# weisongwen/ToySLAM

Hardware: AMD Instinct MI355X
Metric: scan registrations/sec (100k-pt src vs 1M-pt target, 30 Newton iters) (higher is better)
Workload: dtype f32; 1 GPU; single 100k-pt source vs 1M-pt target, 1.0 m voxels, DIRECT7, 30 Newton passes (max_iterations 28, epsilon 1e-9), set U; target_points=1000000, search=DIRECT7, outer_passes=30

## Files before the change

include/ndt_mi355.h:

```cpp
#ifndef NDT_MI355_H_
#define NDT_MI355_H_

#include <stddef.h>
#include <stdint.h>

#ifdef __cplusplus
extern "C" {
#endif

typedef struct ndt_context* ndt_handle;

typedef enum {
  NDT_OK = 0,
  NDT_ERR_INVALID = 1,
  NDT_ERR_NO_DEVICE = 2,
  NDT_ERR_HIP = 3,
  NDT_ERR_GRID_OVERFLOW = 4,
  NDT_ERR_NO_INPUT = 5,
  NDT_ERR_COMM = 6
} ndt_status;

typedef enum { NDT_KDTREE = 0, NDT_DIRECT26 = 1, NDT_DIRECT7 = 2, NDT_DIRECT1 = 3 } ndt_search_method;

const char* ndt_last_error(void);
// ... 112 lines not shown
ndt_status ndt_pcd_read_xyz(const char* path, void* out, size_t capacity_points, size_t stride_bytes, size_t* n_points,
                            int* is_dense);
ndt_status ndt_pcd_write_xyz(const char* path, const void* pts, size_t n, size_t stride_bytes, int binary);

typedef struct ndt_pcd_sequence* ndt_pcd_sequence_handle;
ndt_status ndt_pcd_sequence_open(const char* directory, ndt_pcd_sequence_handle* out);
ndt_status ndt_pcd_sequence_poll(ndt_pcd_sequence_handle s, size_t loaded_clouds, size_t* n_new_files);
ndt_status ndt_pcd_sequence_next(ndt_pcd_sequence_handle s, const void** pts, size_t* n, int* is_dense, int* file_number);
ndt_status ndt_pcd_sequence_stage(ndt_pcd_sequence_handle s, int device);
ndt_status ndt_pcd_sequence_next_device(ndt_pcd_sequence_handle s, const void** d_pts, const void** host_pts, size_t* n, int* is_dense,
                                        int* file_number);
ndt_status ndt_pcd_sequence_next_cloud(ndt_pcd_sequence_handle s, ndt_cloud* cloud, const void** host_pts, size_t* n, int* is_dense,
                                       int* file_number);
void ndt_pcd_sequence_close(ndt_pcd_sequence_handle s);
int ndt_host_extract_file_number(const char* file_stem);
ndt_status ndt_host_repack_fields(const void* data, size_t n, size_t point_step, size_t off_x, size_t off_y, size_t off_z,
                                  void* out_xyz1, int* is_dense);

ndt_status ndt_align_batch(ndt_handle h, const void* pts, const size_t* offsets , size_t n_scans,
                           size_t stride_bytes, const float* guesses ,
                           float* final_transformations , int* has_converged,
                           int* final_num_iteration, double* transformation_probability);
ndt_status ndt_align_batch_device(ndt_handle h, const void* d_pts, const size_t* offsets, size_t n_scans,
                                  size_t stride_bytes, const float* guesses, float* final_transformations,
                                  int* has_converged, int* final_num_iteration, double* transformation_probability);

ndt_status ndt_set_batch_groups(ndt_handle h, int n_groups);

ndt_status ndt_align_pairs(ndt_handle h, const void* pts, const size_t* offsets , size_t n_clouds,
                           size_t stride_bytes, int is_dense, const int* pairs , size_t n_pairs,
                           const float* guesses , float* final_transformations ,
                           int* has_converged, int* final_num_iteration, double* transformation_probability);
ndt_status ndt_align_pairs_clouds(ndt_handle h, const ndt_cloud* clouds, size_t n_clouds, int is_dense, const int* pairs,
                                  size_t n_pairs, const float* guesses, float* final_transformations, int* has_converged,
                                  int* final_num_iteration, double* transformation_probability);
ndt_status ndt_pairs_grid_size(ndt_handle h, size_t cloud, size_t* n_leaves, size_t* n_valid);
ndt_status ndt_pairs_grid_info(ndt_handle h, size_t cloud, int* min_b , int* max_b , int* div_b );
ndt_status ndt_pairs_grid_dump(ndt_handle h, size_t cloud, int64_t* idx, int* nr_points, double* mean, double* cov,
                               double* icov, double* evals);
ndt_status ndt_pairs_fitness_scores(ndt_handle h, const float* transforms , double max_range,
                                    double* fitness );
ndt_status ndt_pairs_count(ndt_handle h, size_t* n_pairs);
ndt_status ndt_batch_fitness_scores(ndt_handle h, const void* pts, const size_t* offsets , size_t n_scans,
                                    size_t stride_bytes, const float* transforms , double max_range,
                                    double* fitness );
ndt_status ndt_batch_fitness_scores_device(ndt_handle h, const void* d_pts, const size_t* offsets, size_t n_scans,
                                           size_t stride_bytes, const float* transforms, double max_range, double* fitness);
ndt_status ndt_diag_fitness_launches(ndt_handle h, size_t* launches, size_t* max_blocks);

ndt_status ndt_grid_centroids(ndt_handle h, float* xyz1 , int64_t* idx , size_t capacity,
                              size_t* n);
ndt_status ndt_grid_centroids_cloud(ndt_handle h, ndt_cloud* out);
ndt_status ndt_get_centroid_fitness_score(ndt_handle h, double max_range, double* fitness);
ndt_status ndt_batch_centroid_fitness_scores(ndt_handle h, const void* pts, const size_t* offsets , size_t n_scans,
                                             size_t stride_bytes, const float* transforms , double max_range,
                                             double* fitness );
ndt_status ndt_batch_centroid_fitness_scores_device(ndt_handle h, const void* d_pts, const size_t* offsets, size_t n_scans,
                                                    size_t stride_bytes, const float* transforms, double max_range, double* fitness);
ndt_status ndt_diag_centroid_fitness(ndt_handle h, size_t* launches, size_t* excursion_passes, float* excursion, size_t* max_blocks);

ndt_status ndt_score_poses(ndt_handle h, const float* transforms , size_t n_poses, double* scores );
ndt_status ndt_diag_score_poses(ndt_handle h, size_t* launches, size_t* blocks);
ndt_status ndt_align_guesses(ndt_handle h, const float* guesses , size_t n_guesses, float* final_transformations,
                             int* has_converged, int* final_num_iteration, double* transformation_probability, int* best);
void ndt_host_pick_top(const double* scores, size_t n, size_t keep, int* idx_out , size_t* n_out);
ndt_status ndt_align_multistart(ndt_handle h, const float* candidates , size_t n_candidates, size_t keep,
                                int* picked, size_t* n_picked, float* final_transformations, int* has_converged,
                                int* final_num_iteration, double* transformation_probability, int* best);

#define NDT_COMM_ID_BYTES 128
ndt_status ndt_comm_get_unique_id(void* id_out );
ndt_status ndt_comm_init_rank(ndt_handle h, const void* id, int rank, int world_size);
ndt_status ndt_comm_destroy(ndt_handle h);
ndt_status ndt_comm_stats(ndt_handle h, int* rank, int* world_size, long long* n_collectives, int* lock_steps);
ndt_status ndt_align_batch_sharded(ndt_handle h, const void* pts, const size_t* offsets , size_t n_local,
                                   size_t first_scan, size_t total_scans, size_t stride_bytes,
                                   const float* guesses , float* final_transformations ,
                                   int* has_converged, int* final_num_iteration, double* transformation_probability);
ndt_status ndt_align_batch_sharded_device(ndt_handle h, const void* d_pts, const size_t* offsets, size_t n_local,
                                          size_t first_scan, size_t total_scans, size_t stride_bytes, const float* guesses,
                                          float* final_transformations, int* has_converged, int* final_num_iteration,
                                          double* transformation_probability);

#define NDT_EVAL_STRIDE 32
typedef int (*ndt_allreduce_fn)(void* buf, size_t n_doubles, int on_device, void* user);
ndt_status ndt_set_allreduce(ndt_handle h, ndt_allreduce_fn fn, void* user, int on_device);

ndt_status ndt_eval(ndt_handle h, const double* p, double* score, double* gradient, double* hessian,
                    double* mean_neighbors);
ndt_status ndt_eval_with_matrix(ndt_handle h, const float* T, const double* p, double* score, double* gradient,
                                double* hessian, double* mean_neighbors);
ndt_status ndt_eval_hessian_f64(ndt_handle h, const double* p, double* hessian);

ndt_status ndt_grid_size(ndt_handle h, size_t* n_leaves, size_t* n_valid);
ndt_status ndt_grid_info(ndt_handle h, int* min_b , int* max_b , int* div_b );
ndt_status ndt_grid_dump(ndt_handle h, int64_t* idx, int* nr_points, double* mean, double* cov, double* icov,
                         double* evals);

ndt_status ndt_profile_enable(ndt_handle h, int on);

ndt_status ndt_set_evaluation_path(ndt_handle h, int persistent);
ndt_status ndt_profile_read(ndt_handle h, int kind, long long* n_launches, double* total_ms, int reset);

ndt_status ndt_selftest_reduce(ndt_handle h, int n_blocks, double* block_sums);
ndt_status ndt_selftest_server_idle(ndt_handle h, const double* p, int stall_ms, int* served_after_stall, double* scores);

ndt_status ndt_diag_stamps(ndt_handle h, const double* p, unsigned long long* stamps, size_t* n_waves);

ndt_status ndt_diag_eval_plan(ndt_handle h, size_t n, int* ppb, int* fused_blocks, int* launch_blocks, int* server_blocks,
                              int* batch_blocks);

ndt_status ndt_host_grid_plan(long long n_cells, long long n_points, const int* div_b , int* bucket_form, int* n_buckets,
                              int* cells_per_bucket, int* pts_per_block, int* n_blocks, int* one_launch, int* wmax, int* lds_cap,
                              long long* lut_cells, int* compact_items, long long* compact_tiles, int* compact_prefix,
                              int* filter_buckets, int* filter_chunks);
ndt_status ndt_diag_grid_build(ndt_handle h, int* form, size_t* n_points, long long* n_cells, int* n_buckets, int* cells_per_bucket,
                               int* pts_per_block, int* n_blocks, int* wmax, int* lds_cap, long long* lut_cells, int* compact_items,
                               long long* compact_tiles, int* compact_prefix, int* compact_pending);

ndt_status ndt_diag_server_roundtrip(ndt_handle h, const double* p, int n_iter, double* us);
ndt_status ndt_diag_selfdrive(ndt_handle h, const double* p, int rounds, double* us);

void ndt_host_solve6(const double* H , const double* b , double* x );
void ndt_host_pose_to_matrix(const double* p , float* T );
void ndt_host_matrix_to_pose(const float* T , double* p );
void ndt_host_angle_derivatives(const double* p , float* j_ang , float* h_ang ,
                                double* j_ang_d , double* h_ang_d );
void ndt_host_gauss(float resolution, double outlier_ratio, double* d );
void ndt_host_thread_budget(int* affinity_cpus, double* quota_cpus, int* local_world_size);
void ndt_host_thread_plan(int affinity_cpus, double quota_cpus, int local_world_size, int* pool_threads, int* max_batch_groups);
typedef int (*ndt_eval_cb)(void* user, int kind, const float* T, const double* p, double* score, double* g, double* H);
ndt_status ndt_host_run_driver(ndt_eval_cb cb, void* user, size_t n_source, const float* guess, float resolution,
                               double step_size, double outlier_ratio, double trans_eps, int max_iter,
                               float* final_transformation, int* has_converged, int* final_num_iteration,
                               double* transformation_probability, int* n_evals, int* n_hessian_recomputes);

#ifdef __cplusplus
}
#endif
#endif
```

toyslam_amd/_lib.py:

```python
import ctypes as C
import os
import subprocess

_HERE = os.path.dirname(os.path.abspath(__file__))
LIB_PATH = os.path.join(_HERE, "libndt_mi355.so")
CSRC = os.path.join(_HERE, "csrc")

NDT_OK, NDT_ERR_INVALID, NDT_ERR_NO_DEVICE, NDT_ERR_HIP, NDT_ERR_GRID_OVERFLOW, NDT_ERR_NO_INPUT, NDT_ERR_COMM = range(7)
KDTREE, DIRECT26, DIRECT7, DIRECT1 = 0, 1, 2, 3
EVAL_STRIDE = 32
COMM_ID_BYTES = 128

ALLREDUCE_FN = C.CFUNCTYPE(C.c_int, C.c_void_p, C.c_size_t, C.c_int, C.c_void_p)
EVAL_CB = C.CFUNCTYPE(C.c_int, C.c_void_p, C.c_int, C.POINTER(C.c_float), C.POINTER(C.c_double),
                      C.POINTER(C.c_double), C.POINTER(C.c_double), C.POINTER(C.c_double))


class NdtError(RuntimeError):
    def __init__(self, status, msg):
        super().__init__("ndt_mi355 status %d: %s" % (status, msg))
        self.status = status


def build(force=False):
# ... 32 lines not shown
    "ndt_set_input_source_device": (C.c_int, [vp, vp, C.c_size_t, C.c_size_t]),
    "ndt_share_input_target": (C.c_int, [vp, vp]),
    "ndt_set_cu_partition": (C.c_int, [vp, C.c_int]),
    "ndt_get_cu_partition": (C.c_int, [vp, ip, ip]),
    "ndt_set_input_target_device_ref": (C.c_int, [vp, vp, C.c_size_t, C.c_int]),
    "ndt_set_input_source_device_ref": (C.c_int, [vp, vp, C.c_size_t]),
    "ndt_share_input_source": (C.c_int, [vp, vp]),
    "ndt_set_voxel_index": (C.c_int, [vp, C.c_int]),
    "ndt_align": (C.c_int, [vp, fp, fp, ip, ip, dp, vp, C.c_size_t]),
    "ndt_get_result": (C.c_int, [vp, fp, ip, ip, dp]),
    "ndt_get_output_device": (C.c_int, [vp, C.POINTER(vp), szp]),
    "ndt_get_stats": (C.c_int, [vp, ip, ip, dp]),
    "ndt_calculate_score": (C.c_int, [vp, vp, C.c_size_t, C.c_size_t, dp]),
    "ndt_voxel_grid_filter": (C.c_int, [vp, vp, C.c_size_t, C.c_size_t, C.c_int, C.c_float, vp, C.c_size_t, szp]),
    "ndt_voxel_grid_filter_device": (C.c_int, [vp, vp, C.c_size_t, C.c_size_t, C.c_int, C.c_float, vp, szp]),
    "ndt_get_fitness_score": (C.c_int, [vp, C.c_double, dp]),
    "ndt_map_clear": (C.c_int, [vp]),
    "ndt_map_update": (C.c_int, [vp, vp, C.c_size_t, C.c_size_t, C.c_int, fp, C.c_float, ip]),
    "ndt_map_update_device": (C.c_int, [vp, vp, C.c_size_t, C.c_size_t, C.c_int, fp, C.c_float, ip]),
    "ndt_map_size": (C.c_int, [vp, szp]),
    "ndt_map_get": (C.c_int, [vp, vp, C.c_size_t]),
    "ndt_map_get_device": (C.c_int, [vp, C.POINTER(C.c_void_p), szp]),
    "ndt_cloud_voxel_filter": (C.c_int, [vp, vp, C.c_size_t, C.c_size_t, C.c_int, C.c_float, C.c_int, C.POINTER(vp), ip]),
    "ndt_warm_up": (C.c_int, [vp, C.c_size_t]),
    "ndt_cloud_upload": (C.c_int, [vp, vp, C.c_size_t, C.c_size_t, C.POINTER(vp)]),
    "ndt_cloud_size": (C.c_int, [vp, szp]),
    "ndt_cloud_data": (C.c_int, [vp, C.POINTER(C.c_void_p), szp]),
    "ndt_cloud_download": (C.c_int, [vp, vp, vp, C.c_size_t]),
    "ndt_cloud_release": (None, [vp]),
    "ndt_set_input_source_cloud": (C.c_int, [vp, vp]),
    "ndt_set_input_target_cloud": (C.c_int, [vp, vp, C.c_int]),
    "ndt_map_update_cloud": (C.c_int, [vp, vp, C.c_int, fp, C.c_float, ip]),
    "ndt_map_update_clouds": (C.c_int, [vp, C.POINTER(vp), C.c_size_t, ip, fp, C.c_float, ip]),
    "ndt_map_update_batch": (C.c_int, [vp, vp, szp, C.c_size_t, C.c_size_t, ip, fp, C.c_float, C.c_int, ip]),
    "ndt_diag_map_batch": (C.c_int, [vp, szp, szp, szp]),
    "ndt_promote_source_to_target": (C.c_int, [vp, C.c_int]),
    "ndt_target_accumulate": (C.c_int, [vp, vp, C.c_size_t, C.c_size_t, C.c_int, fp]),
    "ndt_target_accumulate_device": (C.c_int, [vp, vp, C.c_size_t, C.c_size_t, C.c_int, fp]),
    "ndt_target_accumulate_cloud": (C.c_int, [vp, vp, C.c_int, fp]),
    "ndt_target_accumulate_clouds": (C.c_int, [vp, C.POINTER(vp), C.c_size_t, C.c_int, fp]),
    "ndt_target_accumulate_reset": (C.c_int, [vp]),
    "ndt_target_accumulated": (C.c_int, [vp, szp, szp, szp]),
    "ndt_diag_target_accumulate": (C.c_int, [vp, szp, szp, ip, ip, szp]),
    "ndt_target_accumulate_crop": (C.c_int, [vp, fp, fp]),
    "ndt_diag_target_crop": (C.c_int, [vp, szp, szp, szp, ip, szp]),
    "ndt_target_accumulate_export": (C.c_int, [vp, fp, fp, vp, C.c_size_t, szp]),
    "ndt_target_accumulate_import": (C.c_int, [vp, vp, C.c_size_t]),
    "ndt_target_accumulate_save": (C.c_int, [vp, fp, fp, C.c_char_p]),
    "ndt_target_accumulate_load": (C.c_int, [vp, C.c_char_p]),
    "ndt_diag_target_export": (C.c_int, [vp, szp, szp, szp]),
    "ndt_host_acc_blob_info": (C.c_int, [vp, C.c_size_t, fp, szp, ip, ip]),
    "ndt_host_acc_blob_checksum": (C.c_int, [vp, C.c_size_t, C.POINTER(C.c_uint64)]),
    "ndt_host_acc_pack_cell": (C.c_int, [C.c_int, C.c_int, C.c_int, C.POINTER(C.c_uint64)]),
    "ndt_host_acc_unpack_cell": (None, [C.c_uint64, ip, ip, ip]),
    "ndt_host_chain_pose": (None, [fp, fp, fp]),
    "ndt_host_lattice": (C.c_int, [C.c_float, fp, fp, ip, ip, ip, C.POINTER(C.c_longlong), C.c_int, C.c_longlong, ip]),
    "ndt_pcd_read_header": (C.c_int, [C.c_char_p, szp, ip, ip]),
    "ndt_pcd_read_xyz": (C.c_int, [C.c_char_p, vp, C.c_size_t, C.c_size_t, szp, ip]),
    "ndt_pcd_write_xyz": (C.c_int, [C.c_char_p, vp, C.c_size_t, C.c_size_t, C.c_int]),
    "ndt_align_batch": (C.c_int, [vp, vp, szp, C.c_size_t, C.c_size_t, fp, fp, ip, ip, dp]),
    "ndt_align_batch_device": (C.c_int, [vp, vp, szp, C.c_size_t, C.c_size_t, fp, fp, ip, ip, dp]),
    "ndt_set_allreduce": (C.c_int, [vp, ALLREDUCE_FN, vp, C.c_int]),
    "ndt_set_batch_groups": (C.c_int, [vp, C.c_int]),
    "ndt_align_pairs": (C.c_int, [vp, vp, szp, C.c_size_t, C.c_size_t, C.c_int, ip, C.c_size_t, fp, fp, ip, ip, dp]),
    "ndt_align_pairs_clouds": (C.c_int, [vp, C.POINTER(vp), C.c_size_t, C.c_int, ip, C.c_size_t, fp, fp, ip, ip, dp]),
    "ndt_pairs_grid_size": (C.c_int, [vp, C.c_size_t, szp, szp]),
    "ndt_pairs_grid_info": (C.c_int, [vp, C.c_size_t, ip, ip, ip]),
    "ndt_pairs_grid_dump": (C.c_int, [vp, C.c_size_t, C.POINTER(C.c_int64), ip, dp, dp, dp, dp]),
    "ndt_pairs_fitness_scores": (C.c_int, [vp, fp, C.c_double, dp]),
    "ndt_pairs_count": (C.c_int, [vp, szp]),
    "ndt_diag_fitness_launches": (C.c_int, [vp, szp, szp]),
    "ndt_batch_fitness_scores": (C.c_int, [vp, vp, szp, C.c_size_t, C.c_size_t, fp, C.c_double, dp]),
    "ndt_batch_fitness_scores_device": (C.c_int, [vp, vp, szp, C.c_size_t, C.c_size_t, fp, C.c_double, dp]),
    "ndt_grid_centroids": (C.c_int, [vp, fp, C.POINTER(C.c_int64), C.c_size_t, szp]),
    "ndt_grid_centroids_cloud": (C.c_int, [vp, C.POINTER(vp)]),
    "ndt_get_centroid_fitness_score": (C.c_int, [vp, C.c_double, dp]),
    "ndt_batch_centroid_fitness_scores": (C.c_int, [vp, vp, szp, C.c_size_t, C.c_size_t, fp, C.c_double, dp]),
    "ndt_batch_centroid_fitness_scores_device": (C.c_int, [vp, vp, szp, C.c_size_t, C.c_size_t, fp, C.c_double, dp]),
    "ndt_diag_centroid_fitness": (C.c_int, [vp, szp, szp, fp, szp]),
    "ndt_score_poses": (C.c_int, [vp, fp, C.c_size_t, dp]),
    "ndt_diag_score_poses": (C.c_int, [vp, szp, szp]),
    "ndt_align_guesses": (C.c_int, [vp, fp, C.c_size_t, fp, ip, ip, dp, ip]),
    "ndt_host_pick_top": (None, [dp, C.c_size_t, C.c_size_t, ip, szp]),
    "ndt_align_multistart": (C.c_int, [vp, fp, C.c_size_t, C.c_size_t, ip, szp, fp, ip, ip, dp, ip]),
    "ndt_align_batch_sharded": (C.c_int, [vp, vp, szp, C.c_size_t, C.c_size_t, C.c_size_t, C.c_size_t, fp, fp, ip, ip, dp]),
    "ndt_align_batch_sharded_device": (C.c_int, [vp, vp, szp, C.c_size_t, C.c_size_t, C.c_size_t, C.c_size_t, fp, fp, ip, ip, dp]),
    "ndt_comm_get_unique_id": (C.c_int, [vp]),
    "ndt_comm_init_rank": (C.c_int, [vp, vp, C.c_int, C.c_int]),
    "ndt_comm_destroy": (C.c_int, [vp]),
    "ndt_comm_stats": (C.c_int, [vp, ip, ip, C.POINTER(C.c_longlong), ip]),
    "ndt_eval": (C.c_int, [vp, dp, dp, dp, dp, dp]),
    "ndt_eval_with_matrix": (C.c_int, [vp, fp, dp, dp, dp, dp, dp]),
    "ndt_eval_hessian_f64": (C.c_int, [vp, dp, dp]),
    "ndt_grid_size": (C.c_int, [vp, szp, szp]),
    "ndt_grid_info": (C.c_int, [vp, ip, ip, ip]),
    "ndt_grid_dump": (C.c_int, [vp, C.POINTER(C.c_int64), ip, dp, dp, dp, dp]),
    "ndt_diag_stamps": (C.c_int, [vp, dp, C.POINTER(C.c_ulonglong), szp]),
    "ndt_diag_eval_plan": (C.c_int, [vp, C.c_size_t, ip, ip, ip, ip, ip]),
    "ndt_host_grid_plan": (C.c_int, [C.c_longlong, C.c_longlong, ip, ip, ip, ip, ip, ip, ip, ip, ip, C.POINTER(C.c_longlong), ip,
                                     C.POINTER(C.c_longlong), ip, ip, ip]),
    "ndt_diag_grid_build": (C.c_int, [vp, ip, szp, C.POINTER(C.c_longlong), ip, ip, ip, ip, ip, ip, C.POINTER(C.c_longlong), ip,
                                      C.POINTER(C.c_longlong), ip, ip]),
    "ndt_diag_server_roundtrip": (C.c_int, [vp, dp, C.c_int, dp]),
    "ndt_diag_selfdrive": (C.c_int, [vp, dp, C.c_int, dp]),
    "ndt_selftest_reduce": (C.c_int, [vp, C.c_int, dp]),
    "ndt_selftest_server_idle": (C.c_int, [vp, dp, C.c_int, ip, dp]),
    "ndt_profile_enable": (C.c_int, [vp, C.c_int]),
    "ndt_set_evaluation_path": (C.c_int, [vp, C.c_int]),
    "ndt_profile_read": (C.c_int, [vp, C.c_int, C.POINTER(C.c_longlong), dp, C.c_int]),
    "ndt_host_solve6": (None, [dp, dp, dp]),
    "ndt_host_pose_to_matrix": (None, [dp, fp]),
    "ndt_host_matrix_to_pose": (None, [fp, dp]),
    "ndt_host_angle_derivatives": (None, [dp, fp, fp, dp, dp]),
    "ndt_host_gauss": (None, [C.c_float, C.c_double, dp]),
    "ndt_host_thread_budget": (None, [ip, dp, ip]),
    "ndt_host_thread_plan": (None, [C.c_int, C.c_double, C.c_int, ip, ip]),
    "ndt_host_run_driver": (C.c_int, [EVAL_CB, vp, C.c_size_t, fp, C.c_float, C.c_double, C.c_double, C.c_double,
                                      C.c_int, fp, ip, ip, dp, ip, ip]),
    "ndt_pcd_sequence_open": (C.c_int, [C.c_char_p, C.POINTER(vp)]),
    "ndt_pcd_sequence_poll": (C.c_int, [vp, C.c_size_t, szp]),
    "ndt_pcd_sequence_next": (C.c_int, [vp, C.POINTER(vp), szp, ip, ip]),
    "ndt_pcd_sequence_close": (None, [vp]),
    "ndt_pcd_sequence_stage": (C.c_int, [vp, C.c_int]),
    "ndt_pcd_sequence_next_cloud": (C.c_int, [vp, C.POINTER(vp), C.POINTER(C.c_void_p), szp, ip, ip]),
    "ndt_cloud_voxel_filter_begin": (C.c_int, [vp, vp, C.c_int, C.c_float]),
    "ndt_cloud_voxel_filter_end": (C.c_int, [vp, C.POINTER(vp), ip]),
    "ndt_cloud_voxel_filter_batch": (C.c_int, [vp, vp, szp, C.c_size_t, C.c_size_t, ip, C.c_float, C.c_int, C.POINTER(vp), ip]),
    "ndt_cloud_voxel_filter_clouds": (C.c_int, [vp, C.POINTER(vp), C.c_size_t, ip, C.c_float, C.POINTER(vp), ip]),
    "ndt_diag_filter_batch": (C.c_int, [vp, szp, szp, szp]),
    "ndt_pcd_sequence_next_device": (C.c_int, [vp, C.POINTER(C.c_void_p), C.POINTER(C.c_void_p), szp, ip, ip]),
    "ndt_host_extract_file_number": (C.c_int, [C.c_char_p]),
    "ndt_host_repack_fields": (C.c_int, [vp, C.c_size_t, C.c_size_t, C.c_size_t, C.c_size_t, C.c_size_t, vp, ip]),
    "gicp_create": (C.c_int, [C.c_int, C.POINTER(vp)]),
    "gicp_destroy": (None, [vp]),
    "gicp_set_correspondence_randomness": (C.c_int, [vp, C.c_int]),
    "gicp_set_rotation_epsilon": (C.c_int, [vp, C.c_double]),
    "gicp_set_maximum_optimizer_iterations": (C.c_int, [vp, C.c_int]),
    "gicp_set_transformation_epsilon": (C.c_int, [vp, C.c_double]),
    "gicp_set_maximum_iterations": (C.c_int, [vp, C.c_int]),
    "gicp_set_max_correspondence_distance": (C.c_int, [vp, C.c_double]),
    "gicp_set_input_target": (C.c_int, [vp, vp, C.c_size_t, C.c_size_t]),
    "gicp_set_input_source": (C.c_int, [vp, vp, C.c_size_t, C.c_size_t]),
    "gicp_set_source_covariances": (C.c_int, [vp, dp, C.c_size_t]),
    "gicp_set_target_covariances": (C.c_int, [vp, dp, C.c_size_t]),
    "gicp_set_input_target_cloud": (C.c_int, [vp, vp]),
    "gicp_set_input_source_cloud": (C.c_int, [vp, vp]),
    "gicp_align_pairs_clouds": (C.c_int, [vp, C.POINTER(vp), C.c_size_t, ip, C.c_size_t, fp, C.c_double, fp, ip, ip, ip, dp]),
    "gicp_align_pairs_lockstep": (C.c_int, [vp, C.POINTER(vp), C.c_size_t, ip, C.c_size_t, fp, C.c_double, fp, ip, ip, ip, dp]),
    "gicp_align_guesses": (C.c_int, [vp, fp, C.c_size_t, C.c_double, fp, ip, ip, ip, dp]),
    "gicp_diag_lockstep": (C.c_int, [vp, szp, szp, szp, szp]),
    "gicp_pairs_covariances": (C.c_int, [vp, C.c_size_t, dp]),
    "gicp_diag_pairs": (C.c_int, [vp, szp, szp, szp]),
    "gicp_diag_pairs_time": (C.c_int, [vp, dp, dp]),
    "gicp_align": (C.c_int, [vp, fp, fp, ip, ip, vp]),
    "gicp_get_result": (C.c_int, [vp, fp, ip, ip]),
    "gicp_get_fitness_score": (C.c_int, [vp, C.c_double, dp]),
    "gicp_get_stats": (C.c_int, [vp, ip, ip, ip, ip]),
    "gicp_covariances": (C.c_int, [vp, C.c_int, dp, ip, fp]),
    "gicp_step_correspond": (C.c_int, [vp, fp, fp, ip, fp, ip]),
    "gicp_step_functor": (C.c_int, [vp, C.c_int, dp, dp, dp]),
    "gicp_diag_plan": (C.c_int, [vp, C.c_size_t, ip]),
    "gicp_host_apply_state": (None, [dp, fp]),
}


def lib():
# ... 19 lines not shown
```

toyslam_amd/csrc/ndt_batch.hip:

```cpp
#include "ndt_internal.hpp"

#include <condition_variable>
#include <dlfcn.h>
#include <sched.h>
#include <rccl/rccl.h>

namespace ndtc {

class StepPool {
 public:
  explicit StepPool(int n_threads) : n_(std::max(1, n_threads)) {
    for (int t = 1; t < n_; t++) workers_.emplace_back([this, t] { loop(t); });
  }
  ~StepPool() {
    stop_.store(true, std::memory_order_release);
    post();
    for (auto& w : workers_) w.join();
  }
  template <class F>
  void run(size_t count, const F& fn) {
    if (n_ == 1 || count < 32) {
      for (size_t i = 0; i < count; i++) fn(i);
      return;
    }
// ... 131 lines not shown
  Rccl* r = rccl();
  return fail(NDT_ERR_COMM, std::string(what) + " failed: " + (r ? r->GetErrorString(e) : "librccl unavailable"));
}

void comm_release(ndt_context* h) {
  if (!h->comm) return;
  if (Rccl* r = rccl()) (void)r->CommDestroy(static_cast<ncclComm_t>(h->comm));
  h->comm = nullptr;
  h->comm_rank = 0;
  h->comm_world = 1;
}

ndt_status comm_allreduce(ndt_context* h, double* d_buf, size_t n) {
  Rccl* r = rccl();
  if (!r || !h->comm) return fail(NDT_ERR_COMM, "no communicator");
  const ncclResult_t e = r->AllReduce(d_buf, d_buf, n, ncclDouble, ncclSum, static_cast<ncclComm_t>(h->comm), h->stream);
  if (e != ncclSuccess) return rccl_fail("ncclAllReduce", e);
  h->comm_collectives++;
  return NDT_OK;
}

static int poll_timeout_s() {
  static const int v = [] { const char* e = getenv("NDT_BATCH_TIMEOUT_S"); return e ? std::max(1, atoi(e)) : 60; }();
  return v;
}

template <class LiveFn>
static ndt_status poll_rows(ndt_context* h, size_t n_rows, unsigned long long seq, const LiveFn& live) {
  const auto t0 = std::chrono::steady_clock::now();
  unsigned spins = 0;
  for (size_t k = 0; k < n_rows; k++) {
    if (!live(k)) continue;
    volatile unsigned long long* flag = reinterpret_cast<volatile unsigned long long*>(h->host_result + k * ndt::kEvalStride) + (ndt::kEvalStride - 1);
    while (__atomic_load_n(flag, __ATOMIC_ACQUIRE) != seq) {
      __builtin_ia32_pause();
      if ((++spins & 0xFFFF) == 0) {
        if (hipStreamQuery(h->stream) != hipErrorNotReady) {
          HIP_TRY(hipStreamSynchronize(h->stream));
          if (__atomic_load_n(flag, __ATOMIC_ACQUIRE) == seq) break;
          return fail(NDT_ERR_HIP, "batch step finished without publishing its results");
        }
        if (std::chrono::steady_clock::now() - t0 > std::chrono::seconds(poll_timeout_s())) {
          if (h->comm) {
            Rccl* r = rccl();
            if (r && r->CommAbort) (void)r->CommAbort(static_cast<ncclComm_t>(h->comm));
            h->comm = nullptr;
            h->comm_rank = 0;
            h->comm_world = 1;
            return fail(NDT_ERR_COMM, "timed out waiting for the exchange step (a rank never joined the all-reduce); communicator aborted");
          }
          return fail(NDT_ERR_HIP, "timed out waiting for the batch step");
        }
      }
    }
  }
  return NDT_OK;
}

}

extern "C" {

static ndt_status align_batch_impl(ndt_handle h, const void* pts, const size_t* offsets, size_t n_local, size_t stride,
                                   bool on_device, const float* guesses, float* final_T, int* conv, int* iters,
                                   double* tprob, size_t first = 0, size_t total = 0) {
  if (!h || !offsets) return fail(NDT_ERR_INVALID, "bad arguments");
  if (!h->grid || !h->target) return fail(NDT_ERR_NO_INPUT, "no input target");
  const bool sharded = total != 0;
  if (!sharded) total = n_local;
  if (first + n_local > total) return fail(NDT_ERR_INVALID, "scan range outside the batch");
  const bool exchange = h->comm != nullptr || h->allreduce != nullptr;
  if (sharded && n_local != total && !exchange)
    return fail(NDT_ERR_COMM, "a sharded batch needs a communicator (ndt_comm_init_rank) or an all-reduce hook");
  if (total == 0) return NDT_OK;
  if (total > 65535) return fail(NDT_ERR_INVALID, "at most 65535 scans per batch");
  for (size_t k = 0; k < n_local; k++)
    if (offsets[k + 1] < offsets[k]) return fail(NDT_ERR_INVALID, "offsets must be non-decreasing");
  ndt_status s = ensure_device(h);
  if (s) return s;
  if (!h->is_batch_worker) {
    s = maybe_compact_records(h, true);
    if (s) return s;
  }
  std::shared_ptr<DeviceCloud> cloud;
  const size_t n_pts = n_local ? offsets[n_local] - offsets[0] : 0;
  const unsigned char* base = n_local ? static_cast<const unsigned char*>(pts) + offsets[0] * stride : nullptr;
  s = upload_cloud(h, base, n_pts, stride, on_device, cloud);
  if (s) return s;
  if (n_local) {
    s = order_cloud(h, cloud.get(), offsets, n_local);
    if (s) return s;
  }
  const bool use_sorted = cloud->n_sorted > 0 && !cloud->scan_counts.empty();
  LockStepMembers m;
  m.pts = use_sorted ? cloud->sorted.p : cloud->pts.p;
  m.offset.resize(n_local);
  m.count.resize(n_local);
  m.n_raw.resize(n_local);
  for (size_t k = 0; k < n_local; k++) {
    m.n_raw[k] = offsets[k + 1] - offsets[k];
    m.offset[k] = static_cast<int>(use_sorted ? cloud->scan_starts[k] : offsets[k] - offsets[0]);
    m.count[k] = static_cast<int>(use_sorted ? cloud->scan_counts[k] : m.n_raw[k]);
  }
  return lock_step(h, m, n_local, guesses, final_T, conv, iters, tprob, first, sharded ? total : 0);
}

}

namespace ndtc {

ndt_status lock_step(ndt_context* h, const LockStepMembers& m, size_t n_local, const float* guesses, float* final_T, int* conv,
                     int* iters, double* tprob, size_t first, size_t total) {
  const bool sharded = total != 0;
  if (!sharded) total = n_local;
  const bool exchange = h->comm != nullptr || h->allreduce != nullptr;
  if (m.views && (sharded || exchange)) return fail(NDT_ERR_INVALID, "per-member grids are not sharded");
  const float4* batch_pts = m.pts;
  ndt_status s = ensure_host_rows(h, total);
  if (s) return s;
  HIP_TRY(h->batch_out.reserve(total * ndt::kEvalStride));
  const ndt::Gauss gs = ndt::gauss_constants(h->resolution, h->outlier_ratio);
  auto is_local = [&](size_t g) { return g >= first && g < first + n_local; };

  auto exchange_rows = [&](const std::function<bool(size_t)>& live) -> ndt_status {
    if (h->comm) {
      ndt_status sc = comm_allreduce(h, h->batch_out.p, total * ndt::kEvalStride);
      if (sc) return sc;
      if (h->profiling) HIP_TRY(hipEventRecord(h->ev_c, h->stream));
      const unsigned long long seq = ++h->eval_seq;
      HIP_TRY(ndt::launch_publish_rows(h->batch_out.p, static_cast<int>(total), h->host_result, seq, h->stream));
      if (h->profiling) HIP_TRY(hipEventRecord(h->ev_d, h->stream));
      return poll_rows(h, total, seq, live);
    }
    if (h->allreduce_on_device) {
      HIP_TRY(hipStreamSynchronize(h->stream));
      if (h->allreduce(h->batch_out.p, total * ndt::kEvalStride, 1, h->allreduce_user)) return fail(NDT_ERR_COMM, "allreduce callback failed");
    }
    HIP_TRY(hipMemcpyAsync(h->host_result, h->batch_out.p, total * ndt::kEvalStride * sizeof(double), hipMemcpyDeviceToHost, h->stream));
    HIP_TRY(hipStreamSynchronize(h->stream));
    if (!h->allreduce_on_device && h->allreduce(h->host_result, total * ndt::kEvalStride, 0, h->allreduce_user))
      return fail(NDT_ERR_COMM, "allreduce callback failed");
    return NDT_OK;
  };

  std::vector<size_t> counts(total, 0);
  for (size_t k = 0; k < n_local; k++) counts[first + k] = m.n_raw[k];
  if (sharded && exchange) {
    std::vector<double> rows(total * ndt::kEvalStride, 0.0);
    for (size_t k = 0; k < n_local; k++) rows[(first + k) * ndt::kEvalStride] = static_cast<double>(counts[first + k]);
    HIP_TRY(hipMemcpyAsync(h->batch_out.p, rows.data(), rows.size() * sizeof(double), hipMemcpyHostToDevice, h->stream));
    HIP_TRY(hipStreamSynchronize(h->stream));
    s = exchange_rows([](size_t) { return true; });
    if (s) return s;
    for (size_t g = 0; g < total; g++) counts[g] = static_cast<size_t>(h->host_result[g * ndt::kEvalStride]);
  }

  std::vector<ndt::ScanSolver> solvers(total);
  const size_t pinned_need = (total * sizeof(ndt::ScanDesc) + 4 * total * sizeof(int) + 15) & ~static_cast<size_t>(15);
  if (pinned_need > h->batch_pinned_bytes) {
    if (h->batch_pinned) (void)hipHostFree(h->batch_pinned);
    h->batch_pinned = nullptr;
    h->batch_pinned_bytes = 0;
    HIP_TRY(hipHostMalloc(&h->batch_pinned, pinned_need, hipHostMallocDefault));
    h->batch_pinned_bytes = pinned_need;
  }
  ndt::ScanDesc* descs = static_cast<ndt::ScanDesc*>(h->batch_pinned);
  int* active = reinterpret_cast<int*>(descs + total);
  std::vector<int> live_kind(total, ndt::EVAL_NONE);
  size_t max_n = 0;
  for (size_t g = 0; g < total; g++) {
    solvers[g].start(guesses ? guesses + 16 * g : nullptr, counts[g], solver_params(h));
    descs[g].offset = 0;
    descs[g].count = 0;
    descs[g].pad = 0;
// ... 175 lines not shown
    if (tprob) tprob[g] = solvers[g].trans_probability;
  }
  return NDT_OK;
}

}

extern "C" {

static ndt_status align_batch_grouped(ndt_handle h, const void* pts, const size_t* offsets, size_t n_scans, size_t stride,
                                      bool on_device, const float* guesses, float* final_T, int* conv, int* iters,
                                      double* tprob) {
  const bool exchange = h && (h->comm != nullptr || h->allreduce != nullptr);
  const size_t groups = batch_group_count(h, n_scans);
  if (!h || !offsets || exchange || groups <= 1 || !h->grid || !h->target || h->profiling)
    return align_batch_impl(h, pts, offsets, n_scans, stride, on_device, guesses, final_T, conv, iters, tprob);
  ndt_status s0 = ensure_device(h);
  if (s0) return s0;
  s0 = maybe_compact_records(h, true);
  if (s0) return s0;
  return run_groups(
      h, n_scans, groups, [&](size_t lo, size_t hi) { return static_cast<double>(offsets[hi] - offsets[lo]); },
      [&](ndt_context* w, size_t lo, size_t hi) {
        return align_batch_impl(w, pts, offsets + lo, hi - lo, stride, on_device, guesses ? guesses + 16 * lo : nullptr,
                                final_T ? final_T + 16 * lo : nullptr, conv ? conv + lo : nullptr, iters ? iters + lo : nullptr,
                                tprob ? tprob + lo : nullptr);
      });
}

}

namespace ndtc {

ndt_status many_poses_checks(const ndt_context* h, const void* table, size_t n, const void* out, const char* what) {
  if (!h) return fail(NDT_ERR_INVALID, "null handle");
  if (n && (!table || !out)) return fail(NDT_ERR_INVALID, std::string("null ") + what);
  if (h->comm || h->allreduce)
    return fail(NDT_ERR_INVALID, "one source under many poses is not sharded: the handle has a communicator or an all-reduce hook");
  return NDT_OK;
}

size_t batch_group_count(const ndt_context* h, size_t n_scans) {
  static const int forced = [] { const char* v = getenv("NDT_BATCH_GROUPS"); return v ? std::max(1, atoi(v)) : 0; }();
  size_t groups = (h && h->batch_groups_wanted > 0) ? static_cast<size_t>(h->batch_groups_wanted)
                  : forced                           ? static_cast<size_t>(forced)
                                                     : (n_scans >= 192 ? 4 : n_scans >= 16 ? 2 : 1);
  groups = std::min(groups, std::max<size_t>(1, n_scans / 4));
  static const int max_groups = [] {
    int aff = 1, lw = 1, mg = 1;
    double quota = 0;
    host_thread_budget(&aff, &quota, &lw);
    host_thread_plan(aff, quota, lw, nullptr, &mg);
    return mg;
  }();
  if (!(h && h->batch_groups_wanted > 0) && !forced) groups = std::min(groups, static_cast<size_t>(max_groups));
  return groups;
}

ndt_status run_groups(ndt_context* h, size_t n_scans, size_t groups, const std::function<double(size_t, size_t)>& pts_of,
                      const std::function<ndt_status(ndt_context*, size_t, size_t)>& run) {
  HIP_TRY(hipStreamSynchronize(h->stream));
  while (h->batch_workers.size() < groups) {
    ndt_context* w = new ndt_context();
    w->device = h->device;
    w->is_batch_worker = true;
    h->batch_workers.push_back(w);
  }
  std::vector<ndt_status> st(groups, NDT_OK);
  std::vector<std::string> msg(groups);
  std::vector<std::thread> threads;
  for (size_t g = 0; g < groups; g++) {
    ndt_context* w = h->batch_workers[g];
    w->resolution = h->resolution;
    w->step_size = h->step_size;
    w->outlier_ratio = h->outlier_ratio;
    w->trans_eps = h->trans_eps;
    w->max_iter = h->max_iter;
    w->search = h->search;
    w->min_pts = h->min_pts;
    w->eig_ratio = h->eig_ratio;
    w->target = h->target;
    w->target_dense = h->target_dense;
    w->grid = h->grid;
    const size_t lo = n_scans * g / groups, hi = n_scans * (g + 1) / groups;
    threads.emplace_back([=, &st, &msg, &run] {
      ndt_status s = run(w, lo, hi);
      st[g] = s;
      if (s) msg[g] = ndt_last_error();
    });
  }
  for (auto& t : threads) t.join();
  for (size_t g = 0; g < groups; g++) {
    ndt_context* w = h->batch_workers[g];
    if (w->stream) (void)hipStreamSynchronize(w->stream);
    w->target.reset();
    w->grid.reset();
  }
  long long ne = 0, nh = 0;
  double nn_w = 0, pts_w = 0;
  int steps = 0;
  for (size_t g = 0; g < groups; g++) {
    ndt_context* w = h->batch_workers[g];
    if (st[g]) return fail(st[g], msg[g]);
    const size_t lo = n_scans * g / groups, hi = n_scans * (g + 1) / groups;
    const double evals_pts = static_cast<double>(w->n_evals) * (hi > lo ? pts_of(lo, hi) / static_cast<double>(hi - lo) : 0.0);
    ne += w->n_evals;
    nh += w->n_hess;
    nn_w += w->mean_neighbors * evals_pts;
    pts_w += evals_pts;
    steps = std::max(steps, w->batch_lock_steps);
  }
  h->n_evals = static_cast<int>(std::min<long long>(ne, INT32_MAX));
  h->n_hess = static_cast<int>(std::min<long long>(nh, INT32_MAX));
  h->mean_neighbors = pts_w > 0 ? nn_w / pts_w : 0.0;
  h->batch_lock_steps = steps;
  h->batch_groups = static_cast<int>(groups);
  return NDT_OK;
}

}

extern "C" {

ndt_status ndt_align_batch(ndt_handle h, const void* pts, const size_t* offsets, size_t n_scans, size_t stride,
                           const float* guesses, float* final_T, int* conv, int* iters, double* tprob) {
  return align_batch_grouped(h, pts, offsets, n_scans, stride, false, guesses, final_T, conv, iters, tprob);
}
ndt_status ndt_align_batch_device(ndt_handle h, const void* pts, const size_t* offsets, size_t n_scans, size_t stride,
                                  const float* guesses, float* final_T, int* conv, int* iters, double* tprob) {
  return align_batch_grouped(h, pts, offsets, n_scans, stride, true, guesses, final_T, conv, iters, tprob);
}
ndt_status ndt_align_batch_sharded(ndt_handle h, const void* pts, const size_t* offsets, size_t n_local, size_t first_scan,
                                   size_t total_scans, size_t stride, const float* guesses, float* final_T, int* conv, int* iters,
                                   double* tprob) {
  if (total_scans == 0) return fail(NDT_ERR_INVALID, "total_scans must be > 0");
  return align_batch_impl(h, pts, offsets, n_local, stride, false, guesses, final_T, conv, iters, tprob, first_scan, total_scans);
}
ndt_status ndt_align_batch_sharded_device(ndt_handle h, const void* d_pts, const size_t* offsets, size_t n_local, size_t first_scan,
                                          size_t total_scans, size_t stride, const float* guesses, float* final_T, int* conv,
                                          int* iters, double* tprob) {
  if (total_scans == 0) return fail(NDT_ERR_INVALID, "total_scans must be > 0");
  return align_batch_impl(h, d_pts, offsets, n_local, stride, true, guesses, final_T, conv, iters, tprob, first_scan, total_scans);
}

ndt_status ndt_align_guesses(ndt_handle h, const float* guesses, size_t n_guesses, float* final_T, int* conv, int* iters,
                             double* tprob, int* best) {
  ndt_status s = many_poses_checks(h, guesses, n_guesses, h, "guesses");
  if (s) return s;
  if (n_guesses > 65535) return fail(NDT_ERR_INVALID, "at most 65535 guesses per call");
  if (n_guesses == 0) {
    if (best) *best = -1;
    return NDT_OK;
  }
  s = ensure_device(h);
  if (s) return s;
  if (!h->grid || !h->target) return fail(NDT_ERR_NO_INPUT, "no input target");
  if (!h->source) return fail(NDT_ERR_NO_INPUT, "no input source");
  s = maybe_compact_records(h, true);
  if (s) return s;
  const DeviceCloud& src = *h->source;
  DeviceCloud view;
  LockStepMembers m;
  m.pts = src.pts.p;
  int count = static_cast<int>(src.n);
  if (src.n_sorted > 0) {
    m.pts = src.sorted.p;
    count = static_cast<int>(src.n_sorted);
  } else if (src.n > 0) {
    view.pts.borrow(src.pts.p, src.n);
    view.n = src.n;
    const size_t offsets[2] = {0, src.n};
    s = order_cloud(h, &view, offsets, 1);
    if (s) return s;
    if (view.n_sorted > 0 && !view.scan_counts.empty()) {
      m.pts = view.sorted.p + view.scan_starts[0];
      count = static_cast<int>(view.scan_counts[0]);
    }
  }
  m.offset.assign(n_guesses, 0);
  m.count.assign(n_guesses, count);
  m.n_raw.assign(n_guesses, src.n);
  std::vector<double> tp(n_guesses, 0.0);
  s = lock_step(h, m, n_guesses, guesses, final_T, conv, iters, tp.data());
  if (s) return s;
  if (tprob) std::memcpy(tprob, tp.data(), n_guesses * sizeof(double));
  if (best) {
    *best = -1;
    for (size_t g = 0; g < n_guesses; g++)
      if (!std::isnan(tp[g]) && (*best < 0 || tp[g] > tp[*best])) *best = static_cast<int>(g);
  }
  return NDT_OK;
}

void ndt_host_pick_top(const double* scores, size_t n, size_t keep, int* idx_out, size_t* n_out) {
  std::vector<int> idx;
  for (size_t i = 0; scores && i < n; i++)
    if (std::isfinite(scores[i])) idx.push_back(static_cast<int>(i));
  const size_t k = std::min(keep, idx.size());
  std::partial_sort(idx.begin(), idx.begin() + k, idx.end(),
                    [&](int a, int b) { return scores[a] > scores[b] || (scores[a] == scores[b] && a < b); });
  for (size_t i = 0; idx_out && i < k; i++) idx_out[i] = idx[i];
  if (n_out) *n_out = k;
}

ndt_status ndt_align_multistart(ndt_handle h, const float* candidates, size_t n_candidates, size_t keep, int* picked,
                                size_t* n_picked, float* final_T, int* conv, int* iters, double* tprob, int* best) {
  ndt_status s = many_poses_checks(h, candidates, n_candidates, h, "candidates");
  if (s) return s;
  if (n_candidates > static_cast<size_t>(std::numeric_limits<int>::max())) return fail(NDT_ERR_INVALID, "too many candidates");
  if (std::min(keep, n_candidates) > 65535) return fail(NDT_ERR_INVALID, "at most 65535 guesses are registered per call");
  if (n_picked) *n_picked = 0;
  if (best) *best = -1;
  if (n_candidates == 0 || keep == 0) return NDT_OK;
  std::vector<double> scores(n_candidates);
  s = ndt_score_poses(h, candidates, n_candidates, scores.data());
  if (s) return s;
  std::vector<int> idx(std::min(keep, n_candidates));
  size_t np = 0;
  ndt_host_pick_top(scores.data(), n_candidates, keep, idx.data(), &np);
  if (np == 0) return NDT_OK;
  std::vector<float> guesses(16 * np);
  for (size_t k = 0; k < np; k++) std::memcpy(guesses.data() + 16 * k, candidates + 16 * static_cast<size_t>(idx[k]), 16 * sizeof(float));
  int b = -1;
  s = ndt_align_guesses(h, guesses.data(), np, final_T, conv, iters, tprob, &b);
  if (s) return s;
// ... 79 lines not shown
```

toyslam_amd/csrc/ndt_clouds.hip:

```cpp
#include "ndt_internal.hpp"

#include <immintrin.h>

namespace ndtc {

static void host_repack_bbox(const unsigned char* src, size_t n, size_t stride, float* dst, float bb_min[2][3], float bb_max[2][3]) {
  __m128 mn0 = _mm_set1_ps(FLT_MAX), mx0 = _mm_set1_ps(-FLT_MAX), mn1 = mn0, mx1 = mx0;
  const __m128 keep_xyz = _mm_castsi128_ps(_mm_set_epi32(0, -1, -1, -1)), one_w = _mm_set_ps(1.0f, 0.0f, 0.0f, 0.0f);
  const __m128 abs_mask = _mm_castsi128_ps(_mm_set1_epi32(0x7fffffff)), inf = _mm_set1_ps(INFINITY);
  auto take = [&](__m128 v, float* out) {
    v = _mm_or_ps(_mm_and_ps(v, keep_xyz), one_w);
    _mm_store_ps(out, v);
    mn0 = _mm_min_ps(v, mn0);
    mx0 = _mm_max_ps(v, mx0);
    if ((_mm_movemask_ps(_mm_cmplt_ps(_mm_and_ps(v, abs_mask), inf)) & 7) == 7) {
      mn1 = _mm_min_ps(v, mn1);
      mx1 = _mm_max_ps(v, mx1);
    }
  };
  const size_t n_wide = (stride >= 16) ? n : (n ? n - 1 : 0);
  for (size_t i = 0; i < n_wide; i++) take(_mm_loadu_ps(reinterpret_cast<const float*>(src + i * stride)), dst + 4 * i);
  for (size_t i = n_wide; i < n; i++) {
    const float* p = reinterpret_cast<const float*>(src + i * stride);
    take(_mm_set_ps(0.0f, p[2], p[1], p[0]), dst + 4 * i);
// ... 173 lines not shown

BBox bbox_of(const DeviceCloud& c, int dense) {
  BBox b;
  const int v = dense ? 0 : 1;
  for (int k = 0; k < 3; k++) {
    b.mn[k] = c.bb_min[v][k];
    b.mx[k] = c.bb_max[v][k];
  }
  return b;
}
ndt_status bbox_compute(ndt_context* h, const float4* d_pts, int n, int dense, BBox& out) {
  const int nb = std::min(1024, (n + 255) / 256);
  DevBuf<float> d_mm;
  HIP_TRY(d_mm.reserve(static_cast<size_t>(nb) * 6));
  HIP_TRY(ndt::launch_bbox(d_pts, n, dense, d_mm.p, nb, h->stream));
  std::vector<float> mm(static_cast<size_t>(nb) * 6);
  HIP_TRY(hipMemcpyAsync(mm.data(), d_mm.p, mm.size() * sizeof(float), hipMemcpyDeviceToHost, h->stream));
  HIP_TRY(hipStreamSynchronize(h->stream));
  for (int k = 0; k < 3; k++) {
    out.mn[k] = FLT_MAX;
    out.mx[k] = -FLT_MAX;
  }
  for (int b = 0; b < nb; b++)
    for (int k = 0; k < 3; k++) {
      out.mn[k] = std::min(out.mn[k], mm[b * 6 + k]);
      out.mx[k] = std::max(out.mx[k], mm[b * 6 + 3 + k]);
    }
  return NDT_OK;
}

ndt_status order_range(ndt_context* h, const float4* d_pts, size_t n, float pitch, float4* d_out, size_t* n_out,
                       const BBox* known_bbox) {
  *n_out = 0;
  if (n == 0) return NDT_OK;
  hipStream_t st = h->stream;
  const int ni = static_cast<int>(n);
  BBox bb;
  if (known_bbox) bb = *known_bbox;
  else { ndt_status sb = bbox_compute(h, d_pts, ni, 0, bb); if (sb) return sb; }
  const float* min_p = bb.mn;
  const float* max_p = bb.mx;
  if (!(min_p[0] <= max_p[0])) return NDT_OK;
  ndt::GridGeom geo{};
  while (ndt::lattice_geometry(pitch, min_p, max_p, geo) != ndt::kLatticeOk || geo.n_cells > 4000000) pitch *= 2.0f;
  static const bool radix_on = [] { const char* v = getenv("NDT_ORDER"); return !v || std::strcmp(v, "chain") != 0; }();
  static const size_t radix_from = [] { const char* v = getenv("NDT_ORDER_RADIX_FROM"); return v ? static_cast<size_t>(std::max(0, atoi(v))) : static_cast<size_t>(65536); }();
  if (radix_on && n >= radix_from && ndt::order_radix_passes(geo.n_cells) <= 3) {
    int digit_bits = 0;
    const size_t words = ndt::order_radix_cntmat_words(geo.n_cells, ni, nullptr, nullptr, &digit_bits);
    const int passes = ndt::order_radix_passes(geo.n_cells);
    DevBuf<unsigned> cntmat, bucket_base, counts;
    DevBuf<float4> tmp;
    HIP_TRY(cntmat.reserve(words));
    HIP_TRY(bucket_base.reserve((static_cast<size_t>(1) << digit_bits) + 1));
    HIP_TRY(counts.reserve(4));
    if (passes > 1) HIP_TRY(tmp.reserve(n));
    HIP_TRY(ndt::launch_order_radix(d_pts, ni, geo, cntmat.p, bucket_base.p, tmp.p, d_out, counts.p, st));
    unsigned kept = 0;
    HIP_TRY(hipMemcpyAsync(&kept, counts.p + (passes - 1), sizeof(kept), hipMemcpyDeviceToHost, st));
    HIP_TRY(hipStreamSynchronize(st));
    *n_out = kept;
    return NDT_OK;
  }
  DevBuf<unsigned> cell_count, totals, rank;
  DevBuf<int> key;
  ChainBufs lv;
  HIP_TRY(cell_count.reserve(static_cast<size_t>(geo.n_cells)));
  HIP_TRY(key.reserve(n));
  HIP_TRY(rank.reserve(n));
  HIP_TRY(hipMemsetAsync(cell_count.p, 0, static_cast<size_t>(geo.n_cells) * sizeof(unsigned), st));
  HIP_TRY(ndt::launch_count(d_pts, ni, 0, geo, key.p, rank.p, cell_count.p, st));
  const size_t n_leaves = std::min<size_t>(n, static_cast<size_t>(geo.n_cells));
  HIP_TRY(totals.reserve(4));
  HIP_TRY(lv.reserve(n_leaves, n));
  if (ndt_status s = chain_scan_scatter(st, cell_count.p, geo.n_cells, 1, key.p, rank.p, ni, lv.out(), totals.p)) return s;
  HIP_TRY(ndt::launch_sort_gather(d_pts, lv.leaf_start.p, lv.leaf_count.p, static_cast<int>(n_leaves), lv.sorted_idx.p, d_out, st, totals.p));
  unsigned tot[3];
  HIP_TRY(hipMemcpyAsync(tot, totals.p, sizeof(tot), hipMemcpyDeviceToHost, st));
  HIP_TRY(hipStreamSynchronize(st));
  *n_out = tot[0];
  return NDT_OK;
}

ndt_status order_batch(ndt_context* h, DeviceCloud* c, const size_t* offsets, size_t n_scans) {
  hipStream_t st = h->stream;
  c->scan_counts.assign(n_scans, 0);
  c->scan_starts.assign(n_scans + 1, 0);
  c->n_sorted = 0;
  if (n_scans == 0 || c->n == 0) return NDT_OK;
  constexpr double kMaxCounters = 32.0e6;
  std::vector<int> off(n_scans + 1);
  size_t max_scan = 0;
  for (size_t k = 0; k <= n_scans; k++) off[k] = static_cast<int>(offsets[k] - offsets[0]);
  for (size_t k = 0; k < n_scans; k++) max_scan = std::max(max_scan, offsets[k + 1] - offsets[k]);
  DevBuf<int> d_off, d_box;
  HIP_TRY(d_off.reserve(n_scans + 1));
  HIP_TRY(d_box.reserve(6 * n_scans));
  std::vector<int> box(6 * n_scans);
  for (size_t k = 0; k < n_scans; k++)
    for (int j = 0; j < 6; j++) box[6 * k + j] = j < 3 ? std::numeric_limits<int>::max() : std::numeric_limits<int>::min();
  HIP_TRY(hipMemcpyAsync(d_off.p, off.data(), (n_scans + 1) * sizeof(int), hipMemcpyHostToDevice, st));
  HIP_TRY(hipMemcpyAsync(d_box.p, box.data(), box.size() * sizeof(int), hipMemcpyHostToDevice, st));
  HIP_TRY(ndt::launch_scan_bboxes(c->pts.p, d_off.p, static_cast<int>(n_scans), static_cast<int>(max_scan), d_box.p, st));
  HIP_TRY(hipMemcpyAsync(box.data(), d_box.p, box.size() * sizeof(int), hipMemcpyDeviceToHost, st));
  HIP_TRY(hipStreamSynchronize(st));
  std::vector<ndt::ScanLattice> lat(n_scans);
  for (size_t k = 0; k < n_scans; k++) {
    ndt::ScanLattice& L = lat[k];
    L = ndt::ScanLattice{};
    if (box[6 * k] > box[6 * k + 3]) continue;
    float mn[3], mx[3];
    for (int j = 0; j < 3; j++) { mn[j] = ndt::scan_bbox_decode(box[6 * k + j]); mx[j] = ndt::scan_bbox_decode(box[6 * k + 3 + j]); }
    for (float pitch = h->resolution;; pitch *= 2.0f) {
      const float inv = 1.0f / pitch;
      double cells = 1;
      int div[3];
      for (int j = 0; j < 3; j++) {
        L.min_b[j] = static_cast<int>(std::floor(mn[j] * inv));
        div[j] = static_cast<int>(std::floor(mx[j] * inv)) - L.min_b[j] + 1;
        cells *= div[j];
      }
      if (cells <= kMaxCounters) {
        L.inv_leaf = inv;
        L.mul1 = div[0];
        L.mul2 = div[0] * div[1];
        L.n_cells = static_cast<int>(cells);
        break;
      }
    }
  }
  DevBuf<unsigned> cell_count, totals, rank, d_starts;
  DevBuf<int> key;
  ChainBufs lv;
  DevBuf<ndt::ScanLattice> d_lat;
  DevBuf<long long> d_bases;
  size_t out_base = 0;
  for (size_t s0 = 0; s0 < n_scans;) {
    size_t ns = 0;
    long long total_cells = 0;
    while (s0 + ns < n_scans && (ns == 0 || static_cast<double>(total_cells + lat[s0 + ns].n_cells) <= kMaxCounters)) {
      lat[s0 + ns].base = total_cells;
      total_cells += lat[s0 + ns].n_cells;
      ns++;
    }
    const size_t first_pt = offsets[s0] - offsets[0], n_pts = offsets[s0 + ns] - offsets[s0];
    if (n_pts == 0 || total_cells == 0) {
      for (size_t k = 0; k < ns; k++) c->scan_starts[s0 + k] = out_base;
      s0 += ns;
      continue;
    }
    const int ni = static_cast<int>(n_pts);
    const float4* in = c->pts.p + first_pt;
    std::vector<int> poff(ns + 1);
    std::vector<long long> bases(ns + 1);
    size_t pass_max = 0;
    for (size_t k = 0; k <= ns; k++) poff[k] = static_cast<int>(offsets[s0 + k] - offsets[s0]);
    for (size_t k = 0; k < ns; k++) {
      pass_max = std::max(pass_max, offsets[s0 + k + 1] - offsets[s0 + k]);
      bases[k] = lat[s0 + k].base;
    }
    bases[ns] = total_cells;
    HIP_TRY(d_off.reserve(ns + 1));
    HIP_TRY(d_lat.reserve(ns));
    HIP_TRY(d_bases.reserve(ns + 1));
    HIP_TRY(d_starts.reserve(ns + 1));
    HIP_TRY(hipMemcpyAsync(d_off.p, poff.data(), (ns + 1) * sizeof(int), hipMemcpyHostToDevice, st));
    HIP_TRY(hipMemcpyAsync(d_lat.p, lat.data() + s0, ns * sizeof(ndt::ScanLattice), hipMemcpyHostToDevice, st));
    HIP_TRY(hipMemcpyAsync(d_bases.p, bases.data(), (ns + 1) * sizeof(long long), hipMemcpyHostToDevice, st));
    HIP_TRY(cell_count.reserve(static_cast<size_t>(total_cells) + 1));
    HIP_TRY(key.reserve(n_pts));
    HIP_TRY(rank.reserve(n_pts));
    HIP_TRY(hipMemsetAsync(cell_count.p, 0, (static_cast<size_t>(total_cells) + 1) * sizeof(unsigned), st));
    HIP_TRY(ndt::launch_count_batch(in, d_off.p, static_cast<int>(ns), static_cast<int>(pass_max), d_lat.p, key.p, rank.p, cell_count.p, st));
    const long long scan_cells = total_cells + 1;
    const size_t n_leaves = std::min<size_t>(n_pts, static_cast<size_t>(scan_cells));
    HIP_TRY(totals.reserve(4));
    HIP_TRY(lv.reserve(n_leaves, n_pts));
    if (ndt_status s = chain_scan(st, cell_count.p, scan_cells, 1, lv.out(), totals.p)) return s;
    unsigned tot[3];
    HIP_TRY(hipMemcpyAsync(tot, totals.p, sizeof(tot), hipMemcpyDeviceToHost, st));
    std::vector<unsigned> starts(ns + 1);
    HIP_TRY(ndt::launch_pick(cell_count.p, d_bases.p, d_starts.p, static_cast<int>(ns + 1), st));
    HIP_TRY(hipMemcpyAsync(starts.data(), d_starts.p, (ns + 1) * sizeof(unsigned), hipMemcpyDeviceToHost, st));
    HIP_TRY(ndt::launch_scatter(key.p, rank.p, ni, cell_count.p, lv.sorted_idx.p, st));
    HIP_TRY(ndt::launch_sort_gather(in, lv.leaf_start.p, lv.leaf_count.p, static_cast<int>(n_leaves), lv.sorted_idx.p, c->sorted.p + out_base, st, totals.p));
    HIP_TRY(hipStreamSynchronize(st));
    for (size_t k = 0; k < ns; k++) {
      c->scan_starts[s0 + k] = out_base + starts[k];
      c->scan_counts[s0 + k] = starts[k + 1] - starts[k];
    }
    out_base += starts[ns];
    c->n_sorted += tot[0];
    s0 += ns;
  }
  c->scan_starts[n_scans] = out_base;
  return NDT_OK;
}

ndt_status order_cloud(ndt_context* h, DeviceCloud* c, const size_t* offsets, size_t n_scans) {
  static const int mode = [] { const char* v = getenv("NDT_SORT_SOURCE"); return v ? (atoi(v) != 0 ? 1 : 0) : -1; }();
  constexpr size_t kOrderFrom = 65536;
  c->n_sorted = 0;
  const bool enabled = mode < 0 ? (offsets != nullptr || c->n >= kOrderFrom) : mode != 0;
  if (!enabled || c->n == 0) return NDT_OK;
  HIP_TRY(c->sorted.reserve(c->n));
  if (!offsets) {
    size_t got = 0;
    const BBox bb = bbox_of(*c, 0);
    ndt_status s = order_range(h, c->pts.p, c->n, h->resolution, c->sorted.p, &got, &bb);
    if (s) return s;
    c->n_sorted = got;
  } else {
    ndt_status s = order_batch(h, c, offsets, n_scans);
    if (s) return s;
  }
  return NDT_OK;
}

ndt_status cloud_use_on(ndt_handle h, DeviceCloud* c) {
  if (c->made_on && c->made_on != h->stream) {
    if (c->device != h->device) return fail(NDT_ERR_INVALID, "the cloud lives on another device");
    if (!DevPool::instance().retired(c->made_on)) HIP_TRY(hipStreamSynchronize(c->made_on));
    if (std::find(c->used_on.begin(), c->used_on.end(), h->stream) == c->used_on.end()) c->used_on.push_back(h->stream);
  }
  return NDT_OK;
}

}

extern "C" {

static ndt_status set_source_impl(ndt_handle h, const void* pts, size_t n, size_t stride, bool on_device, bool by_ref = false) {
  if (!h) return fail(NDT_ERR_INVALID, "null handle");
  std::shared_ptr<DeviceCloud> c;
  ndt_status s = upload_cloud(h, pts, n, stride, on_device, c, by_ref);
  if (s) return s;
  s = order_cloud(h, c.get(), nullptr, 0);
  if (s) return s;
  h->source = c;
  return NDT_OK;
}
ndt_status ndt_set_input_source(ndt_handle h, const void* pts, size_t n, size_t stride) {
  return set_source_impl(h, pts, n, stride, false);
}
ndt_status ndt_set_input_source_device(ndt_handle h, const void* pts, size_t n, size_t stride) {
  return set_source_impl(h, pts, n, stride, true);
}
ndt_status ndt_set_input_source_device_ref(ndt_handle h, const void* d_pts, size_t n) {
  return set_source_impl(h, d_pts, n, sizeof(float4), true, true);
}

ndt_status ndt_share_input_source(ndt_handle dst, ndt_handle src) {
  if (!dst || !src) return fail(NDT_ERR_INVALID, "null handle");
  if (!src->source) return fail(NDT_ERR_NO_INPUT, "the donor handle has no input source");
  if (dst == src) return NDT_OK;
  if (dst->device != src->device) return fail(NDT_ERR_INVALID, "handles on different devices");
  HIP_TRY(hipSetDevice(src->device));
  if (src->device_ready) HIP_TRY(hipStreamSynchronize(src->stream));
  ndt_status s = ensure_device(dst);
  if (s) return s;
  HIP_TRY(hipStreamSynchronize(dst->stream));
  dst->source = src->source;
  return NDT_OK;
}

ndt_status ndt_cloud_upload(ndt_handle h, const void* pts, size_t n, size_t stride, ndt_cloud* out) {
  if (!h || !out) return fail(NDT_ERR_INVALID, "bad arguments");
  *out = nullptr;
  std::shared_ptr<DeviceCloud> c;
  ndt_status s = upload_cloud(h, pts, n, stride, false, c);
  if (s) return s;
  c->device = h->device;
  c->made_on = h->stream;
  *out = new ndt_cloud_s{c};
  return NDT_OK;
}

ndt_status ndt_cloud_size(ndt_cloud c, size_t* n) {
  if (!c || !n) return fail(NDT_ERR_INVALID, "bad arguments");
  *n = c->c->n;
  return NDT_OK;
}
ndt_status ndt_cloud_data(ndt_cloud c, const void** d_pts, size_t* n) {
  if (!c || !d_pts || !n) return fail(NDT_ERR_INVALID, "bad arguments");
  *d_pts = c->c->pts.p;
  *n = c->c->n;
  return NDT_OK;
}
ndt_status ndt_cloud_download(ndt_handle h, ndt_cloud c, void* out, size_t out_stride) {
  if (!h || !c || (c->c->n && !out)) return fail(NDT_ERR_INVALID, "bad arguments");
  if (out_stride < 16) return fail(NDT_ERR_INVALID, "out_stride_bytes must be >= 16");
  ndt_status s = ensure_device(h);
  if (!s) s = cloud_use_on(h, c->c.get());
  if (s) return s;
  return download_records(h, c->c->pts.p, c->c->n, out, out_stride);
}
void ndt_cloud_release(ndt_cloud c) { delete c; }

ndt_status ndt_set_input_source_cloud(ndt_handle h, ndt_cloud c) {
// ... 22 lines not shown
```

toyslam_amd/csrc/ndt_grid_kernels.hip:

```cpp
#include "ndt_device.hpp"
#include "ndt_voxel_finish.hpp"

namespace ndt {

namespace {

__global__ __launch_bounds__(kBlock) void k_repack(const unsigned char* __restrict__ src, size_t n, size_t stride,
                                                   float4* __restrict__ dst) {
  for (size_t i = blockIdx.x * (size_t)kBlock + threadIdx.x; i < n; i += (size_t)gridDim.x * kBlock) {
    const float* p = reinterpret_cast<const float*>(src + i * stride);
    dst[i] = make_float4(p[0], p[1], p[2], 1.0f);
  }
}

__global__ __launch_bounds__(kBlock) void k_bbox(const float4* __restrict__ pts, int n, int dense,
                                                 float* __restrict__ block_minmax) {
  float mn[3] = {FLT_MAX, FLT_MAX, FLT_MAX}, mx[3] = {-FLT_MAX, -FLT_MAX, -FLT_MAX};
  for (int i = blockIdx.x * kBlock + threadIdx.x; i < n; i += gridDim.x * kBlock) {
    const float4 p = pts[i];
    if (!dense && !finite3(p.x, p.y, p.z)) continue;
    mn[0] = fminf(mn[0], p.x); mx[0] = fmaxf(mx[0], p.x);
    mn[1] = fminf(mn[1], p.y); mx[1] = fmaxf(mx[1], p.y);
    mn[2] = fminf(mn[2], p.z); mx[2] = fmaxf(mx[2], p.z);
  }
// ... 681 lines not shown
  if (lane == kWave - 1) lds[wave] = inc;
  __syncthreads();
  unsigned base = 0, total = 0;
  for (int w = 0; w < nthreads / kWave; w++) {
    if (w < wave) base += lds[w];
    total += lds[w];
  }
  unsigned run = base + inc - sum;
  for (int i = lo; i < hi; i++) {
    const unsigned v = agent_loads ? __hip_atomic_load(src + i, __ATOMIC_RELAXED, __HIP_MEMORY_SCOPE_AGENT) : src[i];
    dst[i] = run;
    run += v;
  }
  if (tid == 0) dst[n] = total;
}

constexpr int kMatchSlots = 256;
__device__ __forceinline__ unsigned wave_rank(int key, bool valid, unsigned long long* mtab, unsigned short* row, int bits) {
  const int lane = threadIdx.x & (kWave - 1);
  unsigned long long* slot = mtab + (key & (kMatchSlots - 1));
  if (valid) (void)__hip_atomic_fetch_or(slot, 1ull << lane, __ATOMIC_RELAXED, __HIP_MEMORY_SCOPE_WORKGROUP);
  const unsigned long long slotmask = valid ? __hip_atomic_load(slot, __ATOMIC_RELAXED, __HIP_MEMORY_SCOPE_WORKGROUP) : 0ull;
  const unsigned old = valid ? row[key] : 0u;
  unsigned long long peers = slotmask;
#pragma unroll
  for (int b = 8; b < 14; b++) {
    if (b < bits) {
      const bool bit = ((key >> b) & 1) != 0;
      const unsigned long long m = __ballot(bit);
      peers &= bit ? m : ~m;
    }
  }
  const unsigned first_of_slot = __builtin_amdgcn_mbcnt_hi(static_cast<unsigned>(slotmask >> 32), __builtin_amdgcn_mbcnt_lo(static_cast<unsigned>(slotmask), 0u));
  if (valid && first_of_slot == 0) __hip_atomic_store(slot, 0ull, __ATOMIC_RELAXED, __HIP_MEMORY_SCOPE_WORKGROUP);
  const unsigned below = __builtin_amdgcn_mbcnt_hi(static_cast<unsigned>(peers >> 32), __builtin_amdgcn_mbcnt_lo(static_cast<unsigned>(peers), 0u));
  if (valid && below == 0) row[key] = static_cast<unsigned short>(old + static_cast<unsigned>(__popcll(peers)));
  return old + below;
}

__global__ __launch_bounds__(kK1Threads) void k1_hist(const float4* __restrict__ pts, int n, int dense, GridGeom g, int map, int K,
                                                      int ppb, unsigned* __restrict__ cntmat, int* __restrict__ lut, long long lut_cells,
                                                      const unsigned* __restrict__ n_dev) {
  extern __shared__ unsigned k1_lds[];
  if (n_dev) n = min(n, static_cast<int>(*n_dev));
  const K1Deal deal(map & 255, map >> 8);
  unsigned* h = k1_lds;
  const int slice = k1_slice(blockIdx.x, gridDim.x);
  const int lo = min(static_cast<long long>(n), static_cast<long long>(slice) * ppb), hi = min(static_cast<long long>(n), static_cast<long long>(lo) + ppb);
  float4 p[8];
#pragma unroll
  for (int u = 0; u < 8; u++) {
    const int i = lo + threadIdx.x + u * kK1Threads;
    p[u] = (i < hi) ? pts[i] : make_float4(NAN, NAN, NAN, 0.f);
  }
  for (int k = threadIdx.x; k < K; k += kK1Threads) h[k] = 0;
  {
    const long long n4 = lut_cells / 4, per = (n4 + gridDim.x - 1) / gridDim.x;
    const long long lo4 = static_cast<long long>(blockIdx.x) * per, hi4 = min(n4, lo4 + per);
    int4* l4 = reinterpret_cast<int4*>(lut);
    for (long long i = lo4 + threadIdx.x; i < hi4; i += kK1Threads) l4[i] = make_int4(kLutEmpty, kLutEmpty, kLutEmpty, kLutEmpty);
    if (blockIdx.x == 0)
      for (long long i = n4 * 4 + threadIdx.x; i < lut_cells; i += kK1Threads) lut[i] = kLutEmpty;
  }
  __syncthreads();
  for (int base = lo + threadIdx.x; base < hi; base += 8 * kK1Threads) {
    if (base != lo + static_cast<int>(threadIdx.x)) {
#pragma unroll
      for (int u = 0; u < 8; u++) {
        const int i = base + u * kK1Threads;
        p[u] = (i < hi) ? pts[i] : make_float4(NAN, NAN, NAN, 0.f);
      }
    }
#pragma unroll
    for (int u = 0; u < 8; u++) {
      const int c = (base + u * kK1Threads < hi) ? key_of(g, p[u], dense) : -1;
      if (c >= 0) atomicAdd(&h[k1_bucket(c, deal)], 1u);
    }
  }
  __syncthreads();
  for (int k = threadIdx.x; k < K; k += kK1Threads) cntmat[static_cast<size_t>(slice) * K + k] = h[k];
}

constexpr int kColCols = 16, kColGroups = kK1Threads / kColCols, kColRows = 32;
__global__ __launch_bounds__(kK1Threads) void k1_colscan(unsigned* __restrict__ cntmat, int B, int K, unsigned* __restrict__ total) {
  __shared__ unsigned s_part[kColGroups][kColCols + 1];
  const int c = threadIdx.x % kColCols, rg = threadIdx.x / kColCols;
  const int col = blockIdx.x * kColCols + c;
  const int R = (B + kColGroups - 1) / kColGroups;
  const int r0 = rg * R;
  unsigned v[kColRows];
  unsigned sum = 0;
#pragma unroll
  for (int i = 0; i < kColRows; i++) {
    const int r = r0 + i;
    v[i] = (i < R && r < B && col < K) ? cntmat[static_cast<size_t>(r) * K + col] : 0u;
  }
#pragma unroll
  for (int i = 0; i < kColRows; i++) sum += v[i];
  s_part[rg][c] = sum;
  __syncthreads();
  unsigned base = 0, all = 0;
  for (int gq = 0; gq < kColGroups; gq++) {
    const unsigned t = s_part[gq][c];
    if (gq < rg) base += t;
    all += t;
  }
#pragma unroll
  for (int i = 0; i < kColRows; i++) {
    const int r = r0 + i;
    if (i < R && r < B && col < K) cntmat[static_cast<size_t>(r) * K + col] = base;
    base += v[i];
  }
  if (rg == 0 && col < K) total[col] = all;
}

__global__ __launch_bounds__(kK1Threads) void k1_scatter(const float4* __restrict__ pts, int n, int dense, GridGeom g, int map, int K,
                                                         int ppb, const unsigned* __restrict__ cntmat, const unsigned* __restrict__ total,
                                                         unsigned* __restrict__ bucket_base, float4* __restrict__ bpts,
                                                         unsigned* __restrict__ counts, unsigned long long* __restrict__ st, int index_form,
                                                         const unsigned* __restrict__ n_dev) {
  extern __shared__ unsigned k1_lds[];
  if (n_dev) n = min(n, static_cast<int>(*n_dev));
  const K1Deal deal(map & 255, map >> 8);
  __shared__ unsigned s_scan[kK1Waves];
  auto mark = [&](int q) {
    if (st && threadIdx.x == 0) st[8 * blockIdx.x + q] = stamp();
  };
  mark(0);
  __shared__ unsigned long long s_mtab[kK1Waves * kMatchSlots];
  unsigned long long* mtab_all = s_mtab;
  unsigned* cursor = k1_lds;
  unsigned short* tot = reinterpret_cast<unsigned short*>(cursor + K + 2);
  unsigned short* tab = tot + K;
  const int lane = threadIdx.x & (kWave - 1), wave = threadIdx.x / kWave;
  const int b = k1_slice(blockIdx.x, gridDim.x);
  const int kbits = k1_key_bits(K);
  const int lo = min(static_cast<long long>(n), static_cast<long long>(b) * ppb), hi = min(static_cast<long long>(n), static_cast<long long>(lo) + ppb);
  float4 p[8];
#pragma unroll
  for (int u = 0; u < 8; u++) {
    const int i = lo + wave * (8 * kWave) + u * kWave + lane;
    p[u] = (i < hi) ? pts[i] : make_float4(NAN, NAN, NAN, 0.f);
  }
  for (int i = threadIdx.x; i < kK1Waves * kMatchSlots; i += kK1Threads) mtab_all[i] = 0ull;
  for (int i = threadIdx.x; i < kK1Waves * K / 2; i += kK1Threads) reinterpret_cast<unsigned*>(tab)[i] = 0u;
  block_scan_array(total, cursor, K, kK1Threads, s_scan, false);
  __syncthreads();
  if (b == 0) {
    for (int k = threadIdx.x; k <= K; k += kK1Threads) bucket_base[k] = cursor[k];
    if (threadIdx.x == 0) counts[0] = cursor[K];
  }
  for (int k = threadIdx.x; k < K; k += kK1Threads) cursor[k] += cntmat[static_cast<size_t>(b) * K + k];
  __syncthreads();
  mark(1);
  unsigned short* row = tab + wave * K;
  unsigned long long* mtab = mtab_all + wave * kMatchSlots;
  for (int r0 = lo; r0 < hi; r0 += kK1Round) {
    int key[8];
    unsigned rk[8];
    if (r0 != lo) {
#pragma unroll
      for (int u = 0; u < 8; u++) {
        const int i = r0 + wave * (8 * kWave) + u * kWave + lane;
        p[u] = (i < hi) ? pts[i] : make_float4(NAN, NAN, NAN, 0.f);
      }
    }
#pragma unroll
    for (int u = 0; u < 8; u++) {
      const int i = r0 + wave * (8 * kWave) + u * kWave + lane;
      const int c = (i < hi) ? key_of(g, p[u], dense) : -1;
      key[u] = (c >= 0) ? k1_bucket(c, deal) : -1;
      rk[u] = 0;
      if (r0 + wave * (8 * kWave) + u * kWave < hi) rk[u] = wave_rank(key[u], key[u] >= 0, mtab, row, kbits);
    }
    __syncthreads();
    if (r0 == lo) mark(2);
    for (int k = threadIdx.x; k < K; k += kK1Threads) {
      unsigned s_ = 0;
#pragma unroll
      for (int w = 0; w < kK1Waves; w++) {
        const unsigned t = tab[w * K + k];
        tab[w * K + k] = static_cast<unsigned short>(s_);
        s_ += t;
      }
      tot[k] = static_cast<unsigned short>(s_);
    }
    __syncthreads();
    if (r0 == lo) mark(3);
#pragma unroll
    for (int u = 0; u < 8; u++) {
      if (key[u] >= 0) {
        const int i = r0 + wave * (8 * kWave) + u * kWave + lane;
        const unsigned pos = cursor[key[u]] + row[key[u]] + rk[u];
        if (index_form) reinterpret_cast<int*>(bpts)[pos] = i;
        else bpts[pos] = make_float4(p[u].x, p[u].y, p[u].z, __int_as_float(i));
      }
    }
    __syncthreads();
    if (r0 == lo) mark(4);
    if (r0 + kK1Round < hi) {
      for (int k = threadIdx.x; k < K; k += kK1Threads) cursor[k] += tot[k];
      for (int i = threadIdx.x; i < kK1Waves * K / 2; i += kK1Threads) reinterpret_cast<unsigned*>(tab)[i] = 0u;
      __syncthreads();
    }
  }
}

struct K1GlobalSrc {
  const float4* __restrict__ p;
  const int* __restrict__ idx;
  __device__ __forceinline__ float4 operator()(unsigned j) const {
    if (idx) {
      const int i = idx[j];
      float4 q = p[i];
      q.w = __int_as_float(i);
      return q;
    }
    return p[j];
  }
};
__device__ __forceinline__ K1GlobalSrc k1_src(const float4* bpts, const float4* cloud, unsigned bb) {
  return cloud ? K1GlobalSrc{cloud, reinterpret_cast<const int*>(bpts) + bb} : K1GlobalSrc{bpts + bb, nullptr};
}
template <class Src>
__device__ __forceinline__ void k1_cell_histogram(const Src& src, unsigned nb, const GridGeom& g,
                                                  const K1Deal& deal, int C, unsigned* cnt) {
  for (int c = threadIdx.x; c < C; c += kBlock) cnt[c] = 0;
  __syncthreads();
  for (unsigned j = threadIdx.x; j < nb; j += kBlock) {
    const float4 p = src(j);
    atomicAdd(&cnt[k1_local(build_cell(g, p.x, p.y, p.z), deal)], 1u);
  }
  __syncthreads();
}

__global__ __launch_bounds__(kBlock) void k1_count(const float4* __restrict__ bpts, GridGeom g, int map, int K, int C, unsigned min_pts,
                                                   const unsigned* __restrict__ bucket_base, unsigned* __restrict__ tot,
                                                   unsigned* __restrict__ ticket, unsigned* __restrict__ occ_base,
                                                   unsigned* __restrict__ cand_base, unsigned* __restrict__ counts, const float4* __restrict__ cloud) {
  extern __shared__ unsigned k1_lds[];
  const K1Deal deal(map & 255, map >> 8);
  __shared__ U3 s_u3[kBlock / kWave];
  __shared__ unsigned s_scan[kBlock / kWave];
  __shared__ int s_last;
  const int k = blockIdx.x;
  const unsigned bb = bucket_base[k], be = bucket_base[k + 1];
  U3 t = {0, 0, 0};
  if (be > bb) {
    k1_cell_histogram(k1_src(bpts, cloud, bb), be - bb, g, deal, C, k1_lds);
    for (int c = threadIdx.x; c < C; c += kBlock) {
      const unsigned v = k1_lds[c];
      t.occ += (v > 0);
      t.cand += (v >= min_pts);
    }
  }
  U3 total;
  block_exclusive_scan(t, total, s_u3);
  if (threadIdx.x == 0) {
    __hip_atomic_store(tot + 2 * k, total.occ, __ATOMIC_RELAXED, __HIP_MEMORY_SCOPE_AGENT);
    __hip_atomic_store(tot + 2 * k + 1, total.cand, __ATOMIC_RELAXED, __HIP_MEMORY_SCOPE_AGENT);
    asm volatile("s_waitcnt vmcnt(0)" ::: "memory");
    s_last = (__hip_atomic_fetch_add(ticket, 1u, __ATOMIC_RELAXED, __HIP_MEMORY_SCOPE_AGENT) == gridDim.x - 1) ? 1 : 0;
  }
  __syncthreads();
  if (!s_last) return;
  {
    const int tid = threadIdx.x, lane = tid & (kWave - 1), wave = tid / kWave;
    const int per = (K + kBlock - 1) / kBlock, lo = tid * per, hi = min(K, lo + per);
    for (int which = 0; which < 2; which++) {
      unsigned* dst = which ? cand_base : occ_base;
      unsigned sum = 0;
      for (int i = lo; i < hi; i++) sum += __hip_atomic_load(tot + 2 * i + which, __ATOMIC_RELAXED, __HIP_MEMORY_SCOPE_AGENT);
      unsigned inc = sum;
#pragma unroll
      for (int off = 1; off < kWave; off <<= 1) {
        const unsigned a = __shfl_up(inc, off, kWave);
        if (lane >= off) inc += a;
      }
      __syncthreads();
      if (lane == kWave - 1) s_scan[wave] = inc;
      __syncthreads();
      unsigned base = 0, all = 0;
// ... 1158 lines not shown
bool filter_buckets_plan(long long n_cells, int n_points, GridBuildPlan& P) {
  if (!grid_build_plan(n_cells, n_points, P)) return false;
  return (P.shift & 255) == 3;
}
size_t filter_buckets_bitmap_words(long long n_cells) { return static_cast<size_t>(((n_cells + 7) / 8 + 3) / 4 + 1); }
hipError_t launch_filter_buckets(const float4* pts, int n, int dense, const GridGeom& g, const GridBuildPlan& P, const GridBuildScratch& S,
                                 int* st_cell, float4* st_cent, unsigned* bitmap_words, unsigned* wprefix, unsigned* counts ,
                                 float4* out, hipStream_t stream) {
  const int K = P.n_buckets, C = P.cells_per_bucket;
  const size_t lds_scatter = (static_cast<size_t>(K) + 2) * sizeof(unsigned) +
                             static_cast<size_t>(K) * sizeof(unsigned short) + static_cast<size_t>(kK1Waves) * K * sizeof(unsigned short);
  if (lds_scatter > kK1MaxDynamicLds || P.n_blocks > kColGroups * kColRows) return hipErrorInvalidValue;
  static bool once = [] {
    (void)hipFuncSetAttribute(reinterpret_cast<const void*>(&k1_scatter), hipFuncAttributeMaxDynamicSharedMemorySize, static_cast<int>(kK1MaxDynamicLds));
    (void)hipFuncSetAttribute(reinterpret_cast<const void*>(&vf_finalize), hipFuncAttributeMaxDynamicSharedMemorySize, static_cast<int>(kK1MaxDynamicLds));
    return true;
  }();
  (void)once;
  unsigned* total = S.cntmat + static_cast<size_t>(P.n_blocks) * K;
  hipLaunchKernelGGL(k1_hist, dim3(P.n_blocks), dim3(kK1Threads), static_cast<size_t>(K) * sizeof(unsigned), stream, pts, n, dense, g, P.shift, K,
                     P.pts_per_block, S.cntmat, static_cast<int*>(nullptr), 0ll, static_cast<const unsigned*>(nullptr));
  hipLaunchKernelGGL(k1_colscan, dim3((K + kColCols - 1) / kColCols), dim3(kK1Threads), 0, stream, S.cntmat, P.n_blocks, K, total);
  hipLaunchKernelGGL(k1_scatter, dim3(P.n_blocks), dim3(kK1Threads), lds_scatter, stream, pts, n, dense, g, P.shift, K, P.pts_per_block, S.cntmat,
                     total, S.bucket_base, S.bpts, counts, static_cast<unsigned long long*>(nullptr), 0, static_cast<const unsigned*>(nullptr));
  const K1FinishLds F = grid_build_finish_lds(C);
  const int wmax = F.wmax, lds_cap = F.lds_cap;
  if (F.bytes > kK1MaxDynamicLds) return hipErrorInvalidValue;
  hipLaunchKernelGGL(vf_finalize, dim3(K), dim3(kBlock), F.bytes, stream, S.bpts, g, P.shift, K, C, lds_cap, wmax, S.bucket_base, st_cell, st_cent,
                     reinterpret_cast<unsigned char*>(bitmap_words), S.bucket_base + K + 1, S.order, static_cast<unsigned>(n));
  const int n_words = static_cast<int>(((g.n_cells + 7) / 8 + 3) / 4);
  const int n_chunks = filter_buckets_chunks(g.n_cells);
  hipLaunchKernelGGL(vf_bitmap_prefix, dim3(n_chunks), dim3(kBlock), 0, stream, bitmap_words, n_words, wprefix, counts);
  hipLaunchKernelGGL(vf_place, dim3(std::max(1, std::min(2048, (n + kBlock - 1) / kBlock))), dim3(kBlock), 0, stream, st_cell, st_cent, counts, bitmap_words,
                     wprefix, out);
  return hipGetLastError();
}

int order_radix_passes(long long n_cells) {
  int bits = 1;
  while ((1ll << bits) < n_cells) bits++;
  return (bits + 10) / 11;
}
size_t order_radix_cntmat_words(long long n_cells, int n, int* n_blocks_out, int* ppb_out, int* digit_bits_out) {
  int bits = 1;
  while ((1ll << bits) < n_cells) bits++;
  const int passes = (bits + 10) / 11, db = (bits + passes - 1) / passes;
  long long ppb = std::max(512, std::min(kK1Round, pow2_ceil((n + 511) / 512)));
  while ((n + ppb - 1) / ppb > kColGroups * kColRows) ppb += kK1Round;
  const int nb = static_cast<int>(((n + ppb - 1) / ppb + 7) / 8 * 8);
  if (n_blocks_out) *n_blocks_out = nb;
  if (ppb_out) *ppb_out = static_cast<int>(ppb);
  if (digit_bits_out) *digit_bits_out = db;
  return (static_cast<size_t>(nb) + 1) * (static_cast<size_t>(1) << db);
}
hipError_t launch_order_radix(const float4* pts, int n, const GridGeom& g, unsigned* cntmat, unsigned* bucket_base, float4* tmp, float4* out,
                              unsigned* counts, hipStream_t stream) {
  int nb = 0, ppb = 0, db = 0;
  (void)order_radix_cntmat_words(g.n_cells, n, &nb, &ppb, &db);
  const int passes = order_radix_passes(g.n_cells), K = 1 << db;
  const size_t lds_scatter = (static_cast<size_t>(K) + 2) * sizeof(unsigned) + static_cast<size_t>(K) * sizeof(unsigned short) +
                             static_cast<size_t>(kK1Waves) * K * sizeof(unsigned short);
  if (passes > 3 || lds_scatter > kK1MaxDynamicLds || nb > kColGroups * kColRows) return hipErrorInvalidValue;
  static bool once = [] {
    (void)hipFuncSetAttribute(reinterpret_cast<const void*>(&k1_scatter), hipFuncAttributeMaxDynamicSharedMemorySize, static_cast<int>(kK1MaxDynamicLds));
    return true;
  }();
  (void)once;
  unsigned* total = cntmat + static_cast<size_t>(nb) * K;
  const float4* in = pts;
  for (int p = 0; p < passes; p++) {
    float4* dst = ((passes - p) & 1) ? out : tmp;
    const int map = (p * db) | (K << 8);
    const unsigned* n_dev = p ? counts + (p - 1) : nullptr;
    hipLaunchKernelGGL(k1_hist, dim3(nb), dim3(kK1Threads), static_cast<size_t>(K) * sizeof(unsigned), stream, in, n, 0, g, map, K, ppb, cntmat,
                       static_cast<int*>(nullptr), 0ll, n_dev);
    hipLaunchKernelGGL(k1_colscan, dim3((K + kColCols - 1) / kColCols), dim3(kK1Threads), 0, stream, cntmat, nb, K, total);
    hipLaunchKernelGGL(k1_scatter, dim3(nb), dim3(kK1Threads), lds_scatter, stream, in, n, 0, g, map, K, ppb, cntmat, total, bucket_base, dst, counts + p,
                       static_cast<unsigned long long*>(nullptr), 0, n_dev);
    in = dst;
  }
  return hipGetLastError();
}

constexpr int kRcPrefixTiles = 2048;
static int rc_items(long long lut_cells) {
  int items = 1;
  while (items < 8 && lut_cells / (static_cast<long long>(kBlock) * items) >= kRcPrefixTiles) items <<= 1;
  return items;
}
int record_compaction_items(long long lut_cells) { return rc_items(lut_cells); }
bool record_compaction_prefix(long long lut_cells) { return record_compaction_tiles(lut_cells) > static_cast<size_t>(kRcPrefixTiles); }
int filter_buckets_chunks(long long n_cells) {
  const int n_words = static_cast<int>(((n_cells + 7) / 8 + 3) / 4);
  return (n_words + kVfChunkWords - 1) / kVfChunkWords;
}
size_t record_compaction_tiles(long long lut_cells) {
  const long long tile = static_cast<long long>(kBlock) * rc_items(lut_cells);
  return static_cast<size_t>((lut_cells + tile - 1) / tile);
}
template <int ITEMS>
static void launch_rc(int n_tiles, hipStream_t stream, int* lut, long long lut_cells, unsigned* tile_sums, const VoxelRec* recs_in,
                      const VoxelSide* cent_in, VoxelRec* recs_out, VoxelSide* cent_out) {
  hipLaunchKernelGGL((k_rc_count<ITEMS>), dim3(n_tiles), dim3(kBlock), 0, stream, lut, lut_cells, tile_sums);
  if (n_tiles > kRcPrefixTiles) {
    hipLaunchKernelGGL(k_rc_scan, dim3(1), dim3(kBlock), 0, stream, tile_sums, n_tiles);
    hipLaunchKernelGGL((k_rc_apply<ITEMS, true>), dim3(n_tiles), dim3(kBlock), 0, stream, lut, lut_cells, tile_sums, recs_in, cent_in, recs_out, cent_out);
  } else {
    hipLaunchKernelGGL((k_rc_apply<ITEMS, false>), dim3(n_tiles), dim3(kBlock), 0, stream, lut, lut_cells, tile_sums, recs_in, cent_in, recs_out, cent_out);
  }
}
hipError_t launch_compact_records(int* lut, long long lut_cells, const VoxelRec* recs_in, const VoxelSide* cent_in, VoxelRec* recs_out,
                                  VoxelSide* cent_out, unsigned* tile_sums, hipStream_t stream) {
  const int n_tiles = static_cast<int>(record_compaction_tiles(lut_cells));
  switch (rc_items(lut_cells)) {
    case 1: launch_rc<1>(n_tiles, stream, lut, lut_cells, tile_sums, recs_in, cent_in, recs_out, cent_out); break;
    case 2: launch_rc<2>(n_tiles, stream, lut, lut_cells, tile_sums, recs_in, cent_in, recs_out, cent_out); break;
    case 4: launch_rc<4>(n_tiles, stream, lut, lut_cells, tile_sums, recs_in, cent_in, recs_out, cent_out); break;
    default: launch_rc<8>(n_tiles, stream, lut, lut_cells, tile_sums, recs_in, cent_in, recs_out, cent_out); break;
  }
  return hipGetLastError();
}

hipError_t launch_grid_leaves(const GridGeom& g, const GridBuildPlan& P, int min_pts, const float4* bpts, const unsigned* bucket_base,
                              unsigned* scratch , int* leaf_cell, unsigned* leaf_start, int* leaf_count, int* leaf_rec,
                              unsigned* counts, const int* lut, hipStream_t stream, const float4* cloud) {
  const int K = P.n_buckets, C = P.cells_per_bucket;
  unsigned* ticket = scratch;
  unsigned* tot = scratch + 2;
  unsigned* occ_base = tot + 2 * K;
  unsigned* cand_base = occ_base + (K + 1);
  hipError_t e = hipMemsetAsync(ticket, 0, 2 * sizeof(unsigned), stream);
  if (e != hipSuccess) return e;
  hipLaunchKernelGGL(k1_count, dim3(K), dim3(kBlock), static_cast<size_t>(C) * sizeof(unsigned), stream, bpts, g, P.shift, K, C,
                     static_cast<unsigned>(min_pts), bucket_base, tot, ticket, occ_base, cand_base, counts, cloud);
  hipLaunchKernelGGL(k1_leaves, dim3(K), dim3(kBlock), static_cast<size_t>(C) * sizeof(unsigned), stream, bpts, g, P.shift, C, min_pts,
                     bucket_base, occ_base, leaf_cell, leaf_start, leaf_count, leaf_rec, lut, cloud);
  return hipGetLastError();
}

hipError_t launch_sort_gather(const float4* pts, const unsigned* leaf_start, const int* leaf_count, int n_leaves,
                              int* sorted_idx, float4* out, hipStream_t stream, const unsigned* d_totals) {
  if (n_leaves == 0) return hipSuccess;
  hipLaunchKernelGGL(k_presort_large, dim3(presort_grid(n_leaves)), dim3(kBlock), 0, stream, pts, leaf_start, leaf_count, n_leaves, d_totals,
                     sorted_idx, out, presort_chunk(n_leaves));
  hipLaunchKernelGGL(k_sort_gather, dim3((n_leaves + kBlock - 1) / kBlock), dim3(kBlock), 0, stream, pts, leaf_start,
                     leaf_count, n_leaves, d_totals, sorted_idx, out);
  return hipGetLastError();
}

hipError_t launch_voxel_centroids(const float4* pts, const unsigned* leaf_start, const int* leaf_count, int n_leaves,
                                  int* sorted_idx, float4* out, hipStream_t stream, const unsigned* d_totals, float4* d_big_pts) {
  if (n_leaves == 0) return hipSuccess;
  if (d_big_pts)
    hipLaunchKernelGGL(k_presort_large, dim3(presort_grid(n_leaves)), dim3(kBlock), 0, stream, pts, leaf_start, leaf_count, n_leaves, d_totals,
                       sorted_idx, d_big_pts, presort_chunk(n_leaves));
  hipLaunchKernelGGL(k_voxel_centroids, dim3((n_leaves + kBlock - 1) / kBlock), dim3(kBlock), 0, stream, pts, leaf_start,
                     leaf_count, n_leaves, d_totals, sorted_idx, out, d_big_pts);
  return hipGetLastError();
}

__global__ __launch_bounds__(kBlock) void k_copy_records(const float4* __restrict__ src, float4* __restrict__ dst, int n) {
  for (int i = blockIdx.x * kBlock + threadIdx.x; i < n; i += gridDim.x * kBlock) dst[i] = src[i];
}
hipError_t launch_copy_records(const float4* src_host_pinned, float4* dst, int n, hipStream_t stream) {
  if (n <= 0) return hipSuccess;
  hipLaunchKernelGGL(k_copy_records, dim3(grid_for(n, 1024)), dim3(kBlock), 0, stream, src_host_pinned, dst, n);
// ... 58 lines not shown
```

toyslam_amd/csrc/ndt_handle.hip:

```cpp
#include "ndt_internal.hpp"

void ndt_context::release_buffers() {
  target.reset();
  source.reset();
  map_scans.clear();
  grid.reset();
  pairs_grids.clear();
  pair_views.release();
  partials.release();
  ticket.release();
  batch_out.release();
  descs.release();
  out_cloud.release();
  staging.release();
  map_pts.release();
  map_alt.release();
  server_dev_mb.release();
  server_counter.release();
  server_dbg.release();
  sp_poses.release();
}

namespace ndtc {

// ... 279 lines not shown
ndt_status ndt_set_num_threads(ndt_handle h, int n) { if (!h) return fail(NDT_ERR_INVALID, "null"); h->num_threads = n; return NDT_OK; }
ndt_status ndt_set_min_points_per_voxel(ndt_handle h, int n) {
  if (!h) return fail(NDT_ERR_INVALID, "null");
  h->min_pts = (n > 2) ? n : 3;
  return NDT_OK;
}
ndt_status ndt_set_cov_eig_value_inflation_ratio(ndt_handle h, double r) { if (!h) return fail(NDT_ERR_INVALID, "null"); h->eig_ratio = r; return NDT_OK; }
float ndt_get_resolution(ndt_handle h) { return h ? h->resolution : 0.f; }
double ndt_get_step_size(ndt_handle h) { return h ? h->step_size : 0.0; }
double ndt_get_outlier_ratio(ndt_handle h) { return h ? h->outlier_ratio : 0.0; }

ndt_status ndt_get_result(ndt_handle h, float* final_transformation, int* has_converged, int* final_num_iteration,
                          double* transformation_probability) {
  if (!h) return fail(NDT_ERR_INVALID, "null handle");
  if (final_transformation) std::memcpy(final_transformation, h->final_T, sizeof(h->final_T));
  if (has_converged) *has_converged = h->converged;
  if (final_num_iteration) *final_num_iteration = h->nr_iterations;
  if (transformation_probability) *transformation_probability = h->trans_probability;
  return NDT_OK;
}

ndt_status ndt_get_stats(ndt_handle h, int* n_evals, int* n_hess, double* mean_neighbors) {
  if (!h) return fail(NDT_ERR_INVALID, "null handle");
  if (n_evals) *n_evals = h->n_evals;
  if (n_hess) *n_hess = h->n_hess;
  if (mean_neighbors) *mean_neighbors = h->mean_neighbors;
  return NDT_OK;
}

ndt_status ndt_set_cu_partition(ndt_handle h, int partition) {
  if (!h || partition < 0 || partition > 2) return fail(NDT_ERR_INVALID, "bad arguments");
  if (h->cu_partition == partition) return NDT_OK;
  const int old_partition = h->cu_partition;
  h->cu_partition = partition;
  if (!h->device_ready) return NDT_OK;
  HIP_TRY(hipSetDevice(h->device));
  ndt_status s = server_stop(h);
  if (s) return s;
  HIP_TRY(hipStreamSynchronize(h->stream));
  const int total = h->cu_total > 0 ? h->cu_total : 256;
  h->partition_stream[old_partition] = h->stream;
  h->stream_masked[old_partition] = h->cu_count != total;
  h->stream = h->partition_stream[partition];
  if (h->stream) {
    h->cu_count = h->stream_masked[partition] ? (partition == 1 ? total - side_cus() : side_cus()) : total;
  } else {
    const int old_count = h->cu_count;
    s = create_stream(h);
    if (s || !h->stream) {
      h->stream = h->partition_stream[old_partition];
      h->cu_partition = old_partition;
      h->cu_count = old_count;
      tls_pool_stream = h->stream;
      return s ? s : fail(NDT_ERR_HIP, "no stream for the CU partition");
    }
    h->stream_masked[partition] = h->cu_count != total;
    h->partition_stream[partition] = h->stream;
  }
  tls_pool_stream = h->stream;
  return s;
}

ndt_status ndt_get_cu_partition(ndt_handle h, int* partition, int* n_cus) {
  if (!h) return fail(NDT_ERR_INVALID, "null handle");
  ndt_status s = ensure_device(h);
  if (s) return s;
  if (partition) *partition = h->cu_partition;
  if (n_cus) *n_cus = h->cu_count;
  return NDT_OK;
}

ndt_status ndt_profile_enable(ndt_handle h, int on) {
  if (!h) return fail(NDT_ERR_INVALID, "null handle");
  if (on) {
    ndt_status s = ensure_device(h);
    if (s) return s;
    if (!h->ev_a) HIP_TRY(hipEventCreate(&h->ev_a));
    if (!h->ev_b) HIP_TRY(hipEventCreate(&h->ev_b));
    if (!h->ev_c) HIP_TRY(hipEventCreate(&h->ev_c));
    if (!h->ev_d) HIP_TRY(hipEventCreate(&h->ev_d));
  }
  h->profiling = on == 1;
  h->profile_server = on == 2;
  return NDT_OK;
}

ndt_status ndt_profile_read(ndt_handle h, int kind, long long* n_launches, double* total_ms, int reset) {
  if (!h || kind < 0 || kind >= ndt_context::kProfSlots) return fail(NDT_ERR_INVALID, "bad arguments");
  if (n_launches) *n_launches = h->prof_n[kind];
  if (total_ms) *total_ms = h->prof_ms[kind];
  if (reset) {
    h->prof_n[kind] = 0;
    h->prof_ms[kind] = 0;
  }
  return NDT_OK;
}

void ndt_host_solve6(const double* H, const double* b, double* x) { ndt::solve6(H, b, x); }
void ndt_host_pose_to_matrix(const double* p, float* T) { ndt::pose_to_matrix(p, T); }
void ndt_host_matrix_to_pose(const float* T, double* p) { ndt::matrix_to_pose(T, p); }
void ndt_host_angle_derivatives(const double* p, float* j_ang, float* h_ang, double* j_ang_d, double* h_ang_d) {
  ndt::AngleDerivs ad;
  ndt::angle_derivatives(p, ad);
  if (j_ang) std::memcpy(j_ang, ad.j, sizeof(ad.j));
  if (h_ang) std::memcpy(h_ang, ad.h, sizeof(ad.h));
  if (j_ang_d) std::memcpy(j_ang_d, ad.jd, sizeof(ad.jd));
  if (h_ang_d) std::memcpy(h_ang_d, ad.hd, sizeof(ad.hd));
}
void ndt_host_gauss(float resolution, double outlier_ratio, double* d) {
  const ndt::Gauss g = ndt::gauss_constants(resolution, outlier_ratio);
  d[0] = g.d1;
  d[1] = g.d2;
  d[2] = g.d3;
}

ndt_status ndt_host_run_driver(ndt_eval_cb cb, void* user, size_t n_source, const float* guess, float resolution,
                               double step_size, double outlier_ratio, double trans_eps, int max_iter,
                               float* final_transformation, int* has_converged, int* final_num_iteration,
                               double* transformation_probability, int* n_evals, int* n_hess) {
  if (!cb) return fail(NDT_ERR_INVALID, "null callback");
  ndt::SolverParams sp;
  sp.resolution = resolution;
  sp.step_size = step_size;
  sp.outlier_ratio = outlier_ratio;
  sp.trans_eps = trans_eps;
  sp.max_iter = max_iter;
  ndt::ScanSolver solver;
  solver.start(guess, n_source, sp);
  while (!solver.done()) {
    const ndt::EvalRequest& rq = solver.request();
    ndt::EvalResult r;
    std::memset(&r, 0, sizeof(r));
    if (cb(user, rq.kind, rq.T, rq.p, &r.score, r.g, r.H)) return fail(NDT_ERR_INVALID, "evaluator callback failed");
    solver.feed(r);
  }
  if (final_transformation) std::memcpy(final_transformation, solver.final_T, 16 * sizeof(float));
  if (has_converged) *has_converged = solver.converged ? 1 : 0;
  if (final_num_iteration) *final_num_iteration = solver.nr_iterations;
  if (transformation_probability) *transformation_probability = solver.trans_probability;
  if (n_evals) *n_evals = solver.n_evals;
  if (n_hess) *n_hess = solver.n_hess;
  return NDT_OK;
}

}
```

toyslam_amd/csrc/ndt_internal.hpp:

```cpp
#pragma once
#include <hip/hip_runtime.h>

#include <algorithm>
#include <atomic>
#include <functional>
#include <thread>
#include <cfloat>
#include <chrono>
#include <cstdlib>
#include <cmath>
#include <cstdio>
#include <cstring>
#include <limits>
#include <map>
#include <set>
#include <mutex>
#include <memory>
#include <string>
#include <tuple>
#include <vector>

#include "gicp_driver.hpp"
#include "gicp_kernels.hpp"
#include "gicp_mi355.h"
// ... 293 lines not shown
  double t_launch = 0, t_wait = 0, t_solver = 0, t_fill = 0, t_gap = 0;
  float final_T[16] = {1, 0, 0, 0, 0, 1, 0, 0, 0, 0, 1, 0, 0, 0, 0, 1};
  int converged = 0, nr_iterations = 0;
  double trans_probability = 0;
  int n_evals = 0, n_hess = 0;
  double mean_neighbors = 0;
  size_t out_n = 0;
  bool server_running = false;
  int server_blocks = 0;
  DevBuf<float4> map_pts;
  DevBuf<float4> map_alt;
  size_t map_n = 0;
  int map_dense = 1;
  DeviceCloud map_boxes;
  bool map_boxes_known = false;
  hipStream_t map_stream = nullptr;
  hipEvent_t map_ready = nullptr;
  bool map_pending = false;
  FilterPending map_filter;
  std::vector<std::shared_ptr<DeviceCloud>> map_scans;
  float* filter_slots = nullptr;
  hipStream_t filter_stream = nullptr;
  bool n1_pending = false;
  FilterPending n1_filter;
  std::shared_ptr<DeviceCloud> n1_in, n1_out;
  int voxel_index = 0;
  int persistent = -1;
  void* server_host_mbs = nullptr;
  bool server_mbs_on_device = false;
  void* server_host_mb = nullptr;
  int server_flip = 0;
  DevBuf<unsigned char> server_dev_mb;
  DevBuf<unsigned> server_counter;
  int server_counter_set = 0;
  DevBuf<unsigned long long> server_dbg;
  bool server_want_dbg = false;
  int cu_count = 0;
  int cu_total = 0;
  int cu_partition = 0;
  bool profiling = false;
  bool profile_server = false;
  bool server_timed = false;
  hipEvent_t ev_a = nullptr, ev_b = nullptr, ev_c = nullptr, ev_d = nullptr;
  static constexpr int kProfSlots = 7;
  long long prof_n[kProfSlots] = {0, 0, 0, 0, 0, 0, 0};
  double prof_ms[kProfSlots] = {0, 0, 0, 0, 0, 0, 0};
  ndt_allreduce_fn allreduce = nullptr;
  void* allreduce_user = nullptr;
  int allreduce_on_device = 0;
  void* comm = nullptr;
  int comm_rank = 0, comm_world = 1;
  long long comm_collectives = 0;
  int batch_lock_steps = 0;
  int batch_groups = 1;
  bool is_batch_worker = false;
  int batch_groups_wanted = 0;
  std::vector<ndt_context*> batch_workers;
  std::vector<std::shared_ptr<DeviceGrid>> pairs_grids;
  std::vector<std::shared_ptr<DeviceCloud>> pairs_sources;
  std::vector<std::shared_ptr<DeviceGrid>> pairs_targets;
  std::vector<float> pairs_T;
  size_t fit_launches = 0, fit_max_blocks = 0;
  DevBuf<ndt::GridView> pair_views;
  void* fb_pinned = nullptr;
  size_t fb_pinned_bytes = 0;
  void* fb_rows = nullptr;
  size_t fb_rows_bytes = 0;
  size_t fb_passes = 0, fb_single = 0, fb_launches = 0;
  void* mb_pinned = nullptr;
  size_t mb_pinned_bytes = 0;
  size_t mb_transform_launches = 0, mb_filters = 0, mb_box_passes = 0;
  void* sp_pinned = nullptr;
  size_t sp_pinned_bytes = 0;
  DevBuf<float> sp_poses;
  size_t sp_launches = 0, sp_blocks = 0;
  std::shared_ptr<ndtc::AccTarget> acc;
  size_t acc_touched = 0, acc_new = 0, acc_launches = 0;
  int acc_relinked = 0, acc_grown = 0;
  size_t crop_kept = 0, crop_removed = 0, crop_points = 0, crop_launches = 0;
  int crop_relinked = 0;
  size_t exp_voxels = 0, exp_points = 0, exp_launches = 0;
  size_t cf_launches = 0, cf_passes = 0, cf_max_blocks = 0;
  float cf_excursion = 0.f;

  ~ndt_context() {
    for (ndt_context* w : batch_workers) delete w;
    batch_workers.clear();
    ndtc::comm_release(this);
    if (stream) {
      (void)hipSetDevice(device);
      (void)hipStreamSynchronize(stream);
      tls_pool_stream = stream;
    }
    if (map_stream) {
      (void)hipStreamSynchronize(map_stream);
      const hipStream_t keep = tls_pool_stream;
      tls_pool_stream = map_stream;
      map_pts.release();
      map_alt.release();
      tls_pool_stream = keep;
      DevPool::instance().forget_stream(map_stream);
      (void)hipStreamDestroy(map_stream);
      if (map_ready) (void)hipEventDestroy(map_ready);
    }
    if (filter_stream) {
      (void)hipStreamSynchronize(filter_stream);
      n1_in.reset();
      n1_out.reset();
      DevPool::instance().forget_stream(filter_stream);
      (void)hipStreamDestroy(filter_stream);
    }
    if (filter_slots) (void)hipHostFree(filter_slots);
    if (fb_pinned) (void)hipHostFree(fb_pinned);
    if (fb_rows) (void)hipHostFree(fb_rows);
    if (mb_pinned) (void)hipHostFree(mb_pinned);
    if (sp_pinned) (void)hipHostFree(sp_pinned);
    acc.reset();
    release_buffers();
    if (host_result) (void)hipHostFree(host_result);
    if (host_pub) (void)hipHostFree(host_pub);
    if (out_pinned) (void)hipHostFree(out_pinned);
    if (bbox_rows) (void)hipHostFree(bbox_rows);
    if (bbox_tagged) (void)hipHostFree(bbox_tagged);
    for (int k = 0; k < kStageSlots; k++) {
      if (stage_host[k]) (void)hipHostFree(stage_host[k]);
      if (stage_done[k]) (void)hipEventDestroy(stage_done[k]);
    }
    if (server_host_mbs) (void)(server_mbs_on_device ? hipFree(server_host_mbs) : hipHostFree(server_host_mbs));
    if (batch_pinned) (void)hipHostFree(batch_pinned);
    if (ev_a) (void)hipEventDestroy(ev_a);
    if (ev_b) (void)hipEventDestroy(ev_b);
    if (ev_c) (void)hipEventDestroy(ev_c);
    if (ev_d) (void)hipEventDestroy(ev_d);
    for (hipStream_t& ps : partition_stream) {
      if (ps && ps != stream) {
        DevPool::instance().forget_stream(ps);
        (void)hipStreamDestroy(ps);
      }
      ps = nullptr;
    }
    if (stream) {
      DevPool::instance().forget_stream(stream);
      (void)hipStreamDestroy(stream);
    }
    tls_pool_stream = nullptr;
  }
  void release_buffers();
};

namespace ndtc {
int usable_devices();
int side_cus();
ndt_status ensure_device(ndt_context* h);
ndt_status ensure_host_rows(ndt_context* h, size_t rows);
ndt::SolverParams solver_params(const ndt_context* h);
ndt_status pinned_at_least(void*& p, size_t& have, size_t bytes, hipStream_t reader);
struct PoolStreamGuard {
  hipStream_t keep;
  explicit PoolStreamGuard(hipStream_t s) : keep(tls_pool_stream) { tls_pool_stream = s; }
  ~PoolStreamGuard() { tls_pool_stream = keep; }
};
ndt_status upload_cloud(ndt_context* h, const void* pts, size_t n, size_t stride, bool on_device,
                        std::shared_ptr<DeviceCloud>& out, bool by_reference = false);
struct BBox {
  float mn[3], mx[3];
};
BBox bbox_of(const DeviceCloud& c, int dense);
ndt_status bbox_compute(ndt_context* h, const float4* d_pts, int n, int dense, BBox& out);
ndt_status order_range(ndt_context* h, const float4* d_pts, size_t n, float pitch, float4* d_out, size_t* n_out,
                       const BBox* known_bbox = nullptr);
ndt_status order_batch(ndt_context* h, DeviceCloud* c, const size_t* offsets, size_t n_scans);
ndt_status order_cloud(ndt_context* h, DeviceCloud* c, const size_t* offsets, size_t n_scans);
ndt_status download_records(ndt_context* h, const float4* d_src, size_t n, void* out, size_t out_stride);
ndt_status out_block_at_least(ndt_context* h, size_t bytes);
void spread_records(const void* src, size_t n, void* out, size_t out_stride);
ndt_status cloud_use_on(ndt_handle h, DeviceCloud* c);
struct ChainOut { int* leaf_cell; unsigned* leaf_start; int *leaf_count, *leaf_rec, *sorted_idx; };
struct ChainBufs {
  DevBuf<int> leaf_cell, leaf_count, leaf_rec, sorted_idx;
  DevBuf<unsigned> leaf_start;
  hipError_t reserve(size_t max_leaves, size_t n_points) {
    for (hipError_t e : {leaf_cell.reserve(max_leaves), leaf_start.reserve(max_leaves), leaf_count.reserve(max_leaves), leaf_rec.reserve(max_leaves), sorted_idx.reserve(n_points)})
      if (e != hipSuccess) return e;
    return hipSuccess;
  }
  ChainOut out() const { return ChainOut{leaf_cell.p, leaf_start.p, leaf_count.p, leaf_rec.p, sorted_idx.p}; }
};
ndt_status chain_scan(hipStream_t st, unsigned* counters, long long n_cells, int min_pts, const ChainOut& o, unsigned* totals);
ndt_status chain_scan_scatter(hipStream_t st, unsigned* counters, long long n_cells, int min_pts, const int* key, const unsigned* rank,
                              int n, const ChainOut& o, unsigned* totals);
ndt_status sparse_index(hipStream_t st, const float4* pts, int n, int dense, const ndt::GridGeom& geo, int min_pts, const ChainOut& o,
                        unsigned* counts);
struct GridSpec {
  float resolution;
  int min_pts;
  double eig_ratio;
  int voxel_index;
  bool dense;
  bool index_only;
};
inline GridSpec grid_spec_of(const ndt_context* h, int is_dense) {
  return GridSpec{h->resolution, h->min_pts, h->eig_ratio, h->voxel_index, is_dense != 0, false};
}
ndt_status build_grid(ndt_context* h, const std::shared_ptr<DeviceCloud>& cloud, const GridSpec& spec, std::shared_ptr<DeviceGrid>& out);
ndt_status build_grids(ndt_context* h, const std::vector<std::shared_ptr<DeviceCloud>>& targets, int is_dense,
                       std::vector<std::shared_ptr<DeviceGrid>>& out, size_t* n_small);
ndt_status grid_size(ndt_context* h, DeviceGrid* g, size_t* n_leaves, size_t* n_valid);
void grid_info(const DeviceGrid* g, int* min_b, int* max_b, int* div_b);
ndt_status grid_dump(ndt_context* h, DeviceGrid* g, int64_t* idx, int* nr_points, double* mean, double* cov, double* icov, double* evals);
ndt_status maybe_compact_records(ndt_context* h, bool eager);
ndt_status grid_counts(ndt_context* h, DeviceGrid* g);
ndt_status ensure_cell2leaf(ndt_context* h, DeviceGrid* g);
ndt_status ensure_indices(ndt_context* h, const std::vector<DeviceGrid*>& grids);
float index_slack(const DeviceGrid* g);
void fill_point_index(const DeviceGrid* g, ndt::PointIndex& ix);
ndt_status fitness_impl(ndt_context* h, const float4* d_src, int n, const float* T_colmajor, double max_range, double* fitness);
ndt_status fitness_against(ndt_context* h, DeviceGrid* g, const float4* d_src, int n, const float* T_colmajor, double max_range,
                           double* fitness);
struct FitnessJob {
  const DeviceGrid* g = nullptr;
  const float4* src = nullptr;
  size_t n = 0;
  const float* T = nullptr;
};
ndt_status fitness_many(ndt_context* h, const std::vector<FitnessJob>& jobs, double max_range, double* out);
inline int fitness_blocks(int n) { return std::max(1, std::min(2048, (n + 31) / 32)); }
ndt_status filter_slots(ndt_handle h, int which, FilterPending& P);
struct FilterRoute {
  enum Kind { kEmpty, kOverflow, kSparse, kDense } kind = kEmpty;
  ndt::GridGeom geo{};
};
FilterRoute filter_route(const ndt_context* h, size_t n, const BBox& bb, float leaf);
bool filter_takes_buckets(long long n_cells, long long n, ndt::GridBuildPlan& plan);
ndt_status voxel_filter_enqueue(ndt_handle h, hipStream_t st, const float4* d_in, size_t n, int is_dense, float leaf, float4* d_out,
                                const BBox& bb, FilterPending& P);
void voxel_filter_finish(const FilterPending& P, size_t* n_out, DeviceCloud* boxes);
ndt_status voxel_filter_device(ndt_handle h, const float4* d_in, size_t n, int is_dense, float leaf, float4* d_out,
                               size_t* n_out, bool* overflow, const BBox* known_bbox = nullptr, DeviceCloud* out_boxes = nullptr);
struct MapScan {
  std::shared_ptr<DeviceCloud> c;
  int dense = 1;
  const float* pose = nullptr;
};
struct MapBatchDiag {
  size_t transform_launches = 0, filters = 0, box_passes = 0;
};
ndt_status map_update_scans(ndt_handle h, const std::vector<MapScan>& scans, float leaf, int* overflowed, MapBatchDiag* diag);
ndt_status map_settle(ndt_handle h);
ndt_status map_complete(ndt_handle h);
bool acc_is_live(const ndt_context* h);
void acc_drop(ndt_context* h);
ndt_status acc_grid_counts(ndt_context* h, DeviceGrid* g);
ndt_status acc_grid_dump(ndt_context* h, int64_t* idx, int* nr_points, double* mean, double* cov, double* icov, double* evals);
void colmajor_to_T12(const float* m, float* T12);
// ... 45 lines not shown
```

toyslam_amd/csrc/ndt_kernels.hpp:

```cpp
#pragma once
#include <hip/hip_runtime.h>

#include <cmath>
#include <cstdint>

namespace ndt {

struct alignas(64) VoxelRec {
  double mean[3];
  float c[6];
  int n;
  int pad;
  float c01c11[2];
};
static_assert(sizeof(VoxelRec) == 64, "VoxelRec must be one 64-B sector");
struct alignas(64) VoxelSide {
  float cx, cy, cz, pad;
  double icov[6];
};
static_assert(sizeof(VoxelSide) == 64, "VoxelSide must be one 64-B sector");

struct GridGeom {
  float leaf[3];
  float inv_leaf[3];
// ... 103 lines not shown
};

constexpr int kEvalStride = 32;
constexpr int kNumAcc = 29;

hipError_t launch_repack(const void* d_src, size_t n, size_t stride_bytes, float4* d_dst, hipStream_t stream);

struct GridBuildPlan {
  int shift, n_buckets, cells_per_bucket, pts_per_block, n_blocks;
};
bool grid_build_plan(long long n_cells, int n_points, GridBuildPlan& plan);
constexpr int kK1MaxBuckets = 8192;
struct GridBuildScratch {
  unsigned* cntmat;
  unsigned* bucket_base;
  float4* bpts;
  unsigned* order;
  unsigned long long* stamps;
  bool index_form;
};
bool filter_buckets_plan(long long n_cells, int n_points, GridBuildPlan& plan);
size_t filter_buckets_bitmap_words(long long n_cells);
hipError_t launch_filter_buckets(const float4* pts, int n, int dense, const GridGeom& g, const GridBuildPlan& plan, const GridBuildScratch& scratch,
                                 int* st_cell, float4* st_cent, unsigned* bitmap_words, unsigned* wprefix, unsigned* counts, float4* out,
                                 hipStream_t stream);
bool grid_build_small_applies(int n_points, const GridBuildPlan& plan);
struct K1FinishLds {
  int wmax, lds_cap;
  size_t bytes;
};
K1FinishLds grid_build_finish_lds(int cells_per_bucket);
struct SmallBuildDesc {
  const float4* pts;
  int n, dense;
  GridGeom g;
  int map, K, C, min_pts;
  double eig_ratio;
  int lds_cap, wmax, list_cap;
  unsigned fin_words;
  int small_finish;
  unsigned* bucket_base;
  float4* bpts;
  int* sorted_idx;
  VoxelRec* recs;
  VoxelSide* centroids;
  int* lut;
  unsigned* scratch;
  unsigned* counts;
};
bool small_build_desc(int n_points, const GridBuildPlan& plan, bool multi, SmallBuildDesc& desc, size_t* lds_bytes);
hipError_t launch_grid_build_small(const SmallBuildDesc& desc, size_t lds_bytes, unsigned long long* stamps ,
                                   hipStream_t stream);
hipError_t launch_grid_build_small_multi(const SmallBuildDesc* d_descs, int n_targets, int max_K, size_t lds_bytes, hipStream_t stream);
hipError_t launch_grid_build_buckets(const float4* pts, int n, int dense, const GridGeom& g, const GridBuildPlan& plan, int min_pts,
                                     double eig_ratio, const GridBuildScratch& scratch, int* sorted_idx, VoxelRec* recs, VoxelSide* centroids,
                                     int* lut, unsigned* counts, hipStream_t stream);
hipError_t launch_grid_leaves(const GridGeom& g, const GridBuildPlan& plan, int min_pts, const float4* bpts, const unsigned* bucket_base,
                              unsigned* scratch , int* leaf_cell, unsigned* leaf_start, int* leaf_count,
                              int* leaf_rec, unsigned* counts, const int* lut, hipStream_t stream, const float4* cloud = nullptr);
size_t record_compaction_tiles(long long lut_cells);
int record_compaction_items(long long lut_cells);
bool record_compaction_prefix(long long lut_cells);
int filter_buckets_chunks(long long n_cells);
hipError_t launch_compact_records(int* lut, long long lut_cells, const VoxelRec* recs_in, const VoxelSide* cent_in, VoxelRec* recs_out,
                                  VoxelSide* cent_out, unsigned* tile_sums, hipStream_t stream);

hipError_t launch_copy_records(const float4* src_host_pinned, float4* dst, int n, hipStream_t stream);
hipError_t launch_repack_bbox(const void* d_src, size_t n, size_t stride_bytes, float4* d_dst, float* d_block_minmax,
                              int n_blocks, hipStream_t stream, unsigned tag = 0, const unsigned* n_dev = nullptr);
hipError_t launch_bbox(const float4* pts, int n, int dense, float* d_block_minmax, int n_blocks, hipStream_t stream);
hipError_t launch_count(const float4* pts, int n, int dense, const GridGeom& g, int* d_key, unsigned* d_rank,
                        unsigned* d_cell_count, hipStream_t stream);
struct ScanLattice {
  float inv_leaf;
  int min_b[3];
  int mul1, mul2;
  int n_cells;
  long long base;
};
hipError_t launch_scan_bboxes(const float4* pts, const int* d_scan_off, int n_scans, int max_scan_points, int* d_out, hipStream_t stream);
float scan_bbox_decode(int v);
hipError_t launch_count_batch(const float4* pts, const int* d_scan_off, int n_scans, int max_scan_points, const ScanLattice* d_lat,
                              int* d_key, unsigned* d_rank, unsigned* d_cell_count, hipStream_t stream);
hipError_t launch_pick(const unsigned* cell_count, const long long* d_bases, unsigned* d_out, int n, hipStream_t stream);
hipError_t launch_scan_reduce(const unsigned* d_cell_count, long long n_cells, int min_pts, unsigned* d_block_sums,
                              int n_tiles, hipStream_t stream);
hipError_t launch_scan_blocks(unsigned* d_block_sums, int n_tiles, unsigned* d_totals, hipStream_t stream);
hipError_t launch_scan_apply(unsigned* d_cell_count_to_cursor, long long n_cells, int min_pts,
                             const unsigned* d_block_sums, int n_tiles, int* d_leaf_cell,
                             unsigned* d_leaf_start, int* d_leaf_count, int* d_leaf_rec, hipStream_t stream);
hipError_t launch_scatter(const int* d_key, const unsigned* d_rank, int n, const unsigned* d_cell_start, int* d_sorted_idx,
                          hipStream_t stream);

struct SegDesc {
  const unsigned char* src;
  float4* dst;
  const unsigned* range;
  unsigned long long n;
  int stride;
  int pad;
};
hipError_t launch_repack_bbox_multi(const SegDesc* d_segs, int n_segs, size_t max_seg_points, unsigned* d_boxes, hipStream_t stream);
float box_word_decode(unsigned w, bool is_min);
struct FilterBatchCloud {
  GridGeom g;
  int first, n;
  int base;
  int dense;
};
hipError_t launch_count_multi(const float4* pts, const FilterBatchCloud* d_clouds, int n_clouds, int max_cloud_points, int* d_key,
                              unsigned* d_rank, unsigned* d_cell_count, hipStream_t stream);
hipError_t launch_leaf_ranges(const int* leaf_cell, const unsigned* d_totals, const FilterBatchCloud* d_clouds, int n_clouds,
                              unsigned* d_out, hipStream_t stream);

size_t sparse_index_temp_bytes(int n);
hipError_t launch_sparse_index(const float4* pts, int n, int dense, const GridGeom& g, int min_pts, void* temp, size_t temp_bytes,
                               unsigned* keys_a, unsigned* keys_b, int* vals_a, unsigned* flags, unsigned* ord, int* leaf_cell,
                               unsigned* leaf_start, int* leaf_count, int* leaf_rec, int* sorted_idx, unsigned* counts,
                               hipStream_t stream);

struct FinalizeDump {
  int* nr_points;
  double* mean;
  double* cov;
  double* icov;
  double* evals;
};
hipError_t launch_finalize(const float4* pts, const int* d_leaf_cell, const unsigned* d_leaf_start,
                           const int* d_leaf_count, const int* d_leaf_rec, int n_leaves, int* d_sorted_idx,
                           int min_pts, double eig_ratio, VoxelRec* d_recs, VoxelSide* d_centroids, int* d_lut, const GridGeom& geom,
                           unsigned* d_n_valid, FinalizeDump dump, hipStream_t stream, const unsigned* d_totals = nullptr,
                           float4* d_big_pts = nullptr );

hipError_t launch_derivatives(const float4* src, int n, const GridView& gv, const EvalParams& P, int search,
                              bool want_hessian, const ScanDesc* descs, const int* active, int n_active, int max_blocks,
                              int n_blocks, double* partials, hipStream_t stream);
int points_per_block(int n, int cus);
int fused_blocks(int n, int cus, bool partition);
int server_blocks(int n, int cus);
hipError_t launch_derivatives_fused(const float4* src, int n, const GridView& gv, const EvalParams& P, int search,
                                    bool want_hessian, int n_blocks, int ppb, double* partials, unsigned* counter, double* out_row,
                                    unsigned long long seq, hipStream_t stream);
constexpr int kPublishSlots = 64;
constexpr int kServerParts = 16;
constexpr int kServerCmdExit = 0x7fffffff;
constexpr int kServerCmdTransformExit = 4;
size_t server_mailbox_bytes();
void server_reset_mailbox(void* host_mailbox);
void server_post(void* host_mailbox, unsigned long long seq, int kind, const float* T12, const double* cos_sin6);
unsigned long long server_dead_word(const void* host_mailbox);
hipError_t launch_selfdrive(const float4* src, int n, const GridView& gv, int search, void* dev_mailbox, int n_blocks, int ppb, double* partials,
                            unsigned* counter, double* parts, double* out_row, unsigned long long first_seq, int rounds, int with_body,
                            double gauss_d1, double gauss_d2, int param_pad, hipStream_t stream);
hipError_t launch_eval_server(const float4* src, int n, const GridView& gv, int search, void* host_mailbox,
                              void* dev_mailbox, int n_blocks, int ppb, double* partials, unsigned* counter, double* out_row,
                              unsigned long long first_seq, unsigned long long idle_ticks, double gauss_d1, double gauss_d2,
                              int param_pad, const float4* out_src, float4* out_dst, int out_n, hipStream_t stream,
                              unsigned long long* dbg, int direct, float4* out_host, unsigned* counter_next);
constexpr int kServerCounterWords = 32 * (1 + kServerParts);
hipError_t launch_hessian64(const float4* src, int n, const GridView& gv, const Hess64Params& P, int search,
                            const ScanDesc* descs, const int* active, int n_active, int max_blocks, int n_blocks,
                            double* partials, hipStream_t stream);
hipError_t launch_reduce(const double* partials, int n_blocks, int n_scans, const ScanDesc* descs, double* out,
                         hipStream_t stream, unsigned long long seq = 0);
hipError_t launch_publish_rows(const double* d_rows, int n_rows, double* host_rows, unsigned long long seq, hipStream_t stream);
hipError_t launch_batch_step(const float4* src, const GridView& gv, int search, const ScanDesc* descs, const int* active,
// ... 48 lines not shown
```

toyslam_amd/ndt.py:

```python
import ctypes as C
import os

import numpy as np

from . import _lib
from ._lib import COMM_ID_BYTES, DIRECT1, DIRECT7, DIRECT26, KDTREE, NdtError, check


def _f(a):
    return a.ctypes.data_as(C.POINTER(C.c_float))


def _d(a):
    return a.ctypes.data_as(C.POINTER(C.c_double))


def _i(a):
    return a.ctypes.data_as(C.POINTER(C.c_int))


def _cloud(a):
    a = np.ascontiguousarray(a, dtype=np.float32)
    if a.ndim != 2 or a.shape[1] < 3:
        raise ValueError("cloud must be (N, >=3)")
# ... 405 lines not shown
    def targetAccumulated(self):
        p, v, u = C.c_size_t(0), C.c_size_t(0), C.c_size_t(0)
        check(self._L.ndt_target_accumulated(self._h, C.byref(p), C.byref(v), C.byref(u)))
        return dict(points=p.value, voxels=v.value, updates=u.value)

    def targetAccumulateDiag(self):
        t, n, l = C.c_size_t(0), C.c_size_t(0), C.c_size_t(0)
        r, g = C.c_int(0), C.c_int(0)
        check(self._L.ndt_diag_target_accumulate(self._h, C.byref(t), C.byref(n), C.byref(r), C.byref(g), C.byref(l)))
        return dict(touched_voxels=t.value, new_voxels=n.value, relinked=bool(r.value), table_grown=bool(g.value), launches=l.value)

    def targetAccumulateCrop(self, min_xyz, max_xyz):
        mn, mx = (np.ascontiguousarray(v, dtype=np.float32).reshape(3) for v in (min_xyz, max_xyz))
        check(self._L.ndt_target_accumulate_crop(self._h, _f(mn), _f(mx)))
        return self.targetAccumulated()

    def targetCropDiag(self):
        k, r, p, l = C.c_size_t(0), C.c_size_t(0), C.c_size_t(0), C.c_size_t(0)
        w = C.c_int(0)
        check(self._L.ndt_diag_target_crop(self._h, C.byref(k), C.byref(r), C.byref(p), C.byref(w), C.byref(l)))
        return dict(kept_voxels=k.value, removed_voxels=r.value, kept_points=p.value, relinked=bool(w.value), launches=l.value)

    @staticmethod
    def _box(min_xyz, max_xyz):
        if (min_xyz is None) != (max_xyz is None):
            raise ValueError("give both bounds, or neither for every voxel")
        if min_xyz is None:
            return None, None
        mn, mx = (np.ascontiguousarray(v, dtype=np.float32).reshape(3) for v in (min_xyz, max_xyz))
        return mn, mx

    def targetAccumulateExport(self, min_xyz=None, max_xyz=None):
        mn, mx = self._box(min_xyz, max_xyz)
        cap = 64 + ACC_ROW_DTYPE.itemsize * self.targetAccumulated()["voxels"]
        buf = np.empty(cap, dtype=np.uint8)
        n = C.c_size_t(0)
        check(self._L.ndt_target_accumulate_export(self._h, _f(mn) if mn is not None else None, _f(mx) if mx is not None else None,
                                                   buf.ctypes.data, cap, C.byref(n)))
        return buf[:n.value].tobytes()

    def targetAccumulateImport(self, blob):
        b = np.frombuffer(bytes(blob), dtype=np.uint8)
        check(self._L.ndt_target_accumulate_import(self._h, b.ctypes.data if len(b) else None, len(b)))
        return self.targetAccumulated()

    def targetAccumulateSave(self, path, min_xyz=None, max_xyz=None):
        mn, mx = self._box(min_xyz, max_xyz)
        check(self._L.ndt_target_accumulate_save(self._h, _f(mn) if mn is not None else None, _f(mx) if mx is not None else None,
                                                 os.fsencode(path)))

    def targetAccumulateLoad(self, path):
        check(self._L.ndt_target_accumulate_load(self._h, os.fsencode(path)))
        return self.targetAccumulated()

    def targetExportDiag(self):
        v, p, l = C.c_size_t(0), C.c_size_t(0), C.c_size_t(0)
        check(self._L.ndt_diag_target_export(self._h, C.byref(v), C.byref(p), C.byref(l)))
        return dict(voxels=v.value, points=p.value, launches=l.value)

    def alignBatch(self, clouds=None, guesses=None, device_ptr=None, offsets=None, stride_bytes=16):
        if clouds is not None:
            cols = {c.shape[1] for c in clouds}
            if len(cols) != 1:
                raise ValueError("all clouds must have the same column count")
            cat = _cloud(np.concatenate(clouds, axis=0))
            offsets = np.zeros(len(clouds) + 1, dtype=np.uintp)
            offsets[1:] = np.cumsum([c.shape[0] for c in clouds])
            ptr, stride, fn = cat.ctypes.data, cat.shape[1] * 4, self._L.ndt_align_batch
        else:
            offsets = np.ascontiguousarray(offsets, dtype=np.uintp)
            ptr, stride, fn = C.c_void_p(device_ptr), stride_bytes, self._L.ndt_align_batch_device
        B = len(offsets) - 1
        g = None
        if guesses is not None:
            g = np.ascontiguousarray(np.stack([_colmajor(x) for x in guesses]))
        T = np.zeros((B, 16), dtype=np.float32)
        conv = np.zeros(B, dtype=np.int32)
        it = np.zeros(B, dtype=np.int32)
        tp = np.zeros(B, dtype=np.float64)
        check(fn(self._h, ptr, offsets.ctypes.data_as(C.POINTER(C.c_size_t)), B, stride,
                 _f(g) if g is not None else None, _f(T), _i(conv), _i(it), _d(tp)))
        return dict(T=np.stack([_from_colmajor(T[k]) for k in range(B)]), converged=conv.astype(bool),
                    iterations=it, trans_probability=tp)

    def alignPairs(self, clouds, pairs=None, guesses=None, is_dense=True):
        resident = [isinstance(c, DeviceCloud) for c in clouds]
        if any(resident) and not all(resident):
            raise ValueError("clouds must be all DeviceCloud or all host arrays, not a mix")
        P = pairs_array(len(clouds), pairs)
        n = P.shape[0]
        g = None
        if guesses is not None:
            g = np.ascontiguousarray(np.stack([_colmajor(x) for x in guesses]))
            if g.shape[0] != n:
                raise ValueError("one guess per pair")
        T = np.zeros((n, 16), dtype=np.float32)
        conv = np.zeros(n, dtype=np.int32)
        it = np.zeros(n, dtype=np.int32)
        tp = np.zeros(n, dtype=np.float64)
        out = (_f(g) if g is not None else None, _f(T), _i(conv), _i(it), _d(tp))
        if clouds and all(isinstance(c, DeviceCloud) for c in clouds):
            arr = (C.c_void_p * len(clouds))(*[c._c for c in clouds])
            check(self._L.ndt_align_pairs_clouds(self._h, arr, len(clouds), int(is_dense), _i(P), n, *out))
        else:
            cols = {np.asarray(c).shape[1] for c in clouds}
            if len(cols) > 1:
                raise ValueError("all clouds must have the same column count")
            cat = _cloud(np.concatenate(clouds, axis=0)) if clouds else np.zeros((0, 4), np.float32)
            offsets = np.zeros(len(clouds) + 1, dtype=np.uintp)
            offsets[1:] = np.cumsum([len(c) for c in clouds])
            check(self._L.ndt_align_pairs(self._h, cat.ctypes.data, offsets.ctypes.data_as(C.POINTER(C.c_size_t)), len(clouds),
                                          cat.shape[1] * 4, int(is_dense), _i(P), n, *out))
        return dict(T=np.stack([_from_colmajor(T[k]) for k in range(n)]) if n else np.zeros((0, 4, 4), np.float32),
                    converged=conv.astype(bool), iterations=it, trans_probability=tp)

    def pairsFitness(self, transforms=None, max_range=np.finfo(np.float64).max):
        T = None
        if transforms is not None:
            T = np.ascontiguousarray(np.stack([_colmajor(x) for x in transforms]), dtype=np.float32)
        n = C.c_size_t(0)
        check(self._L.ndt_pairs_count(self._h, C.byref(n)))
        P = n.value
        if T is not None and T.shape[0] != P:
            raise ValueError("one transform per pair of the last alignPairs")
        out = np.zeros(max(P, 1), dtype=np.float64)
        check(self._L.ndt_pairs_fitness_scores(self._h, _f(T) if T is not None else None, float(max_range), _d(out)))
        return out[:P].copy()

    def fitnessLaunches(self):
        a, b = C.c_size_t(0), C.c_size_t(0)
        check(self._L.ndt_diag_fitness_launches(self._h, C.byref(a), C.byref(b)))
        return a.value, b.value

    def batchFitness(self, clouds=None, transforms=None, max_range=np.finfo(np.float64).max, device_ptr=None, offsets=None,
                     stride_bytes=16):
        if clouds is not None:
            cat = _cloud(np.concatenate(clouds, axis=0)) if len(clouds) else np.zeros((0, 4), np.float32)
            offsets = np.zeros(len(clouds) + 1, dtype=np.uintp)
            offsets[1:] = np.cumsum([len(c) for c in clouds])
            ptr, stride, fn = cat.ctypes.data, cat.shape[1] * 4, self._L.ndt_batch_fitness_scores
        else:
            offsets = np.ascontiguousarray(offsets, dtype=np.uintp)
            ptr, stride, fn = C.c_void_p(device_ptr), stride_bytes, self._L.ndt_batch_fitness_scores_device
        B = len(offsets) - 1
        if transforms is None:
            raise ValueError("batchFitness needs one transform per scan")
        T = np.ascontiguousarray(np.stack([_colmajor(x) for x in transforms]), dtype=np.float32) if B else np.zeros((0, 16), np.float32)
        if T.shape[0] != B:
            raise ValueError("one transform per scan")
        out = np.zeros(max(B, 1), dtype=np.float64)
        check(fn(self._h, ptr, offsets.ctypes.data_as(C.POINTER(C.c_size_t)), B, stride, _f(T) if B else None, float(max_range),
                 _d(out)))
        return out[:B].copy()

    def gridCentroids(self):
        n = C.c_size_t(0)
        check(self._L.ndt_grid_centroids(self._h, None, None, 0, C.byref(n)))
        V = n.value
        xyz1 = np.zeros((max(V, 1), 4), dtype=np.float32)
        idx = np.zeros(max(V, 1), dtype=np.int64)
        if V:
            check(self._L.ndt_grid_centroids(self._h, _f(xyz1), idx.ctypes.data_as(C.POINTER(C.c_int64)), V, C.byref(n)))
        return xyz1[:V].copy(), idx[:V].copy()

    def gridCentroidsCloud(self):
        c = C.c_void_p(None)
# ... 535 lines not shown
```

Before: 2222 registrations/s.

## Order batch scans with multi-pass LSD radix sort reading device input directly

Replaces the chained counting-sort ordering of batched scans with a per-member multi-pass radix sort (histogram, column scan, scatter), planned from cell counts. When input is already on device as aligned float4, ordering reads the source directly and skips the upload copy. It also adds optional prepare-phase timing and a diagnostic batch-order API. The workload is a single-scan registration dominated by 30 Newton iterations, so this batch-preparation path may barely affect the measured loop.

```diff
diff --git a/include/ndt_mi355.h b/include/ndt_mi355.h
--- a/include/ndt_mi355.h
+++ b/include/ndt_mi355.h
@@ -218,6 +218,11 @@
                                           float* final_transformations, int* has_converged, int* final_num_iteration,
                                           double* transformation_probability);
 
+ndt_status ndt_diag_batch_order(ndt_handle h, const void* pts, const size_t* offsets, size_t n_scans, size_t stride_bytes, int on_device,
+                                float resolution, void* ordered, size_t* starts, size_t* counts, size_t* n_ordered);
+void ndt_host_order_batch_plan(long long max_cells, size_t max_member_points, size_t total_points, int* passes, int* digit_bits,
+                               int* points_per_block);
+
 #define NDT_EVAL_STRIDE 32
 typedef int (*ndt_allreduce_fn)(void* buf, size_t n_doubles, int on_device, void* user);
 ndt_status ndt_set_allreduce(ndt_handle h, ndt_allreduce_fn fn, void* user, int on_device);
diff --git a/toyslam_amd/_lib.py b/toyslam_amd/_lib.py
--- a/toyslam_amd/_lib.py
+++ b/toyslam_amd/_lib.py
@@ -138,6 +138,8 @@
     "ndt_diag_score_poses": (C.c_int, [vp, szp, szp]),
     "ndt_align_guesses": (C.c_int, [vp, fp, C.c_size_t, fp, ip, ip, dp, ip]),
     "ndt_host_pick_top": (None, [dp, C.c_size_t, C.c_size_t, ip, szp]),
+    "ndt_diag_batch_order": (C.c_int, [vp, vp, szp, C.c_size_t, C.c_size_t, C.c_int, C.c_float, vp, szp, szp, szp]),
+    "ndt_host_order_batch_plan": (None, [C.c_longlong, C.c_size_t, C.c_size_t, ip, ip, ip]),
     "ndt_align_multistart": (C.c_int, [vp, fp, C.c_size_t, C.c_size_t, ip, szp, fp, ip, ip, dp, ip]),
     "ndt_align_batch_sharded": (C.c_int, [vp, vp, szp, C.c_size_t, C.c_size_t, C.c_size_t, C.c_size_t, fp, fp, ip, ip, dp]),
     "ndt_align_batch_sharded_device": (C.c_int, [vp, vp, szp, C.c_size_t, C.c_size_t, C.c_size_t, C.c_size_t, fp, fp, ip, ip, dp]),
diff --git a/toyslam_amd/csrc/ndt_batch.hip b/toyslam_amd/csrc/ndt_batch.hip
--- a/toyslam_amd/csrc/ndt_batch.hip
+++ b/toyslam_amd/csrc/ndt_batch.hip
@@ -237,14 +237,30 @@
     s = maybe_compact_records(h, true);
     if (s) return s;
   }
+  static const bool prepare_env = [] { const char* v = getenv("NDT_PROFILE_PREPARE"); return v && atoi(v) != 0; }();
+  const bool time_prepare = h->profile_prepare || prepare_env;
+  const auto prepare_t0 = std::chrono::steady_clock::now();
+  if (time_prepare) {
+    if (!h->ev_p0) HIP_TRY(hipEventCreate(&h->ev_p0));
+    if (!h->ev_p1) HIP_TRY(hipEventCreate(&h->ev_p1));
+    HIP_TRY(hipEventRecord(h->ev_p0, h->stream));
+  }
   std::shared_ptr<DeviceCloud> cloud;
   const size_t n_pts = n_local ? offsets[n_local] - offsets[0] : 0;
   const unsigned char* base = n_local ? static_cast<const unsigned char*>(pts) + offsets[0] * stride : nullptr;
-  s = upload_cloud(h, base, n_pts, stride, on_device, cloud);
-  if (s) return s;
-  if (n_local) {
-    s = order_cloud(h, cloud.get(), offsets, n_local);
-    if (s) return s;
+  s = batch_cloud(h, base, n_pts, stride, on_device, offsets, n_local, h->resolution, cloud);
+  if (s) return s;
+  if (time_prepare) {
+    HIP_TRY(hipEventRecord(h->ev_p1, h->stream));
+    HIP_TRY(hipEventSynchronize(h->ev_p1));
+    float ms = 0;
+    HIP_TRY(hipEventElapsedTime(&ms, h->ev_p0, h->ev_p1));
+    const double host_ms = std::chrono::duration<double, std::milli>(std::chrono::steady_clock::now() - prepare_t0).count();
+    h->prep_n[0]++;
+    h->prep_ms[0] += ms;
+    h->prep_n[1]++;
+    h->prep_ms[1] += host_ms;
+    if (prepare_env) std::fprintf(stderr, "[batch prepare] scans %zu points %zu device_ms %.4f host_ms %.4f\n", n_local, n_pts, ms, host_ms);
   }
   const bool use_sorted = cloud->n_sorted > 0 && !cloud->scan_counts.empty();
   LockStepMembers m;
@@ -586,6 +602,7 @@
     w->target = h->target;
     w->target_dense = h->target_dense;
     w->grid = h->grid;
+    w->profile_prepare = h->profile_prepare;
     const size_t lo = n_scans * g / groups, hi = n_scans * (g + 1) / groups;
     threads.emplace_back([=, &st, &msg, &run] {
       ndt_status s = run(w, lo, hi);
@@ -606,6 +623,12 @@
   for (size_t g = 0; g < groups; g++) {
     ndt_context* w = h->batch_workers[g];
     if (st[g]) return fail(st[g], msg[g]);
+    for (int k = 0; k < 2; k++) {
+      h->prep_n[k] += w->prep_n[k];
+      h->prep_ms[k] += w->prep_ms[k];
+      w->prep_n[k] = 0;
+      w->prep_ms[k] = 0;
+    }
     const size_t lo = n_scans * g / groups, hi = n_scans * (g + 1) / groups;
     const double evals_pts = static_cast<double>(w->n_evals) * (hi > lo ? pts_of(lo, hi) / static_cast<double>(hi - lo) : 0.0);
     ne += w->n_evals;
@@ -645,6 +668,38 @@
                                           int* iters, double* tprob) {
   if (total_scans == 0) return fail(NDT_ERR_INVALID, "total_scans must be > 0");
   return align_batch_impl(h, d_pts, offsets, n_local, stride, true, guesses, final_T, conv, iters, tprob, first_scan, total_scans);
+}
+
+ndt_status ndt_diag_batch_order(ndt_handle h, const void* pts, const size_t* offsets, size_t n_scans, size_t stride, int on_device,
+                                float resolution, void* ordered, size_t* starts, size_t* counts, size_t* n_ordered) {
+  if (!h || !offsets || !n_ordered) return fail(NDT_ERR_INVALID, "bad arguments");
+  if (!(resolution > 0)) return fail(NDT_ERR_INVALID, "resolution must be > 0");
+  if (n_scans > 65535) return fail(NDT_ERR_INVALID, "at most 65535 scans per batch");
+  for (size_t k = 0; k < n_scans; k++)
+    if (offsets[k + 1] < offsets[k]) return fail(NDT_ERR_INVALID, "offsets must be non-decreasing");
+  *n_ordered = 0;
+  ndt_status s = ensure_device(h);
+  if (s) return s;
+  std::shared_ptr<DeviceCloud> cloud;
+  const size_t n_pts = n_scans ? offsets[n_scans] - offsets[0] : 0;
+  const unsigned char* base = n_scans ? static_cast<const unsigned char*>(pts) + offsets[0] * stride : nullptr;
+  s = batch_cloud(h, base, n_pts, stride, on_device != 0, offsets, n_scans, resolution, cloud);
+  if (s) return s;
+  const bool sorted = cloud->n_sorted > 0 && !cloud->scan_counts.empty();
+  for (size_t k = 0; k < n_scans; k++) {
+    if (starts) starts[k] = sorted ? cloud->scan_starts[k] : 0;
+    if (counts) counts[k] = sorted ? cloud->scan_counts[k] : 0;
+  }
+  if (starts) starts[n_scans] = sorted ? cloud->scan_starts[n_scans] : 0;
+  *n_ordered = sorted ? cloud->n_sorted : 0;
+  if (sorted && ordered) return download_records(h, cloud->sorted.p, cloud->n_sorted, ordered, sizeof(float4));
+  HIP_TRY(hipStreamSynchronize(h->stream));
+  return NDT_OK;
+}
+
+void ndt_host_order_batch_plan(long long max_cells, size_t max_member_points, size_t total_points, int* passes, int* digit_bits,
+                               int* points_per_block) {
+  ndt::order_batch_radix_plan(max_cells, max_member_points, total_points, passes, digit_bits, points_per_block);
 }
 
 ndt_status ndt_align_guesses(ndt_handle h, const float* guesses, size_t n_guesses, float* final_T, int* conv, int* iters,
diff --git a/toyslam_amd/csrc/ndt_clouds.hip b/toyslam_amd/csrc/ndt_clouds.hip
--- a/toyslam_amd/csrc/ndt_clouds.hip
+++ b/toyslam_amd/csrc/ndt_clouds.hip
@@ -279,7 +279,67 @@
   return NDT_OK;
 }
 
-ndt_status order_batch(ndt_context* h, DeviceCloud* c, const size_t* offsets, size_t n_scans) {
+static bool order_radix_on() {
+  static const bool on = [] { const char* v = getenv("NDT_ORDER"); return !v || std::strcmp(v, "chain") != 0; }();
+  return on;
+}
+static ndt_status order_batch_chain(ndt_context* h, DeviceCloud* c, const float4* src, const size_t* offsets, size_t n_scans,
+                                    std::vector<ndt::ScanLattice>& lat, double kMaxCounters);
+
+static ndt_status order_batch_radix(ndt_context* h, DeviceCloud* c, const float4* src, const size_t* offsets, size_t n_scans,
+                                    const std::vector<ndt::ScanLattice>& lat, size_t max_scan, bool w_one) {
+  hipStream_t st = h->stream;
+  long long max_cells = 0;
+  for (size_t k = 0; k < n_scans; k++) max_cells = std::max<long long>(max_cells, lat[k].n_cells);
+  if (max_cells == 0) return NDT_OK;
+  int passes = 0, db = 0, ppb = 0;
+  ndt::order_batch_radix_plan(max_cells, max_scan, c->n, &passes, &db, &ppb);
+  std::vector<ndt::OrderMember> mem(n_scans);
+  auto lay_out = [&] {
+    unsigned long long words = 0;
+    for (size_t k = 0; k < n_scans; k++) {
+      ndt::OrderMember& M = mem[k];
+      M.lat = lat[k];
+      M.in_off = static_cast<int>(offsets[k] - offsets[0]);
+      M.n = static_cast<int>(offsets[k + 1] - offsets[k]);
+      M.nb = static_cast<int>((static_cast<size_t>(M.n) + ppb - 1) / ppb);
+      M.cnt_off = words;
+      words += (static_cast<unsigned long long>(M.nb) + 1) << db;
+    }
+    return words;
+  };
+  unsigned long long words = lay_out();
+  const int bits = passes * db;
+  while (words > (1ull << 26) && db > 4) {
+    passes++;
+    db = std::max(4, (bits + passes - 1) / passes);
+    words = lay_out();
+  }
+  int max_nb = 0;
+  for (const ndt::OrderMember& M : mem) max_nb = std::max(max_nb, M.nb);
+  DevBuf<ndt::OrderMember> d_mem;
+  DevBuf<unsigned> cntmat, d_res;
+  DevBuf<float4> tmp;
+  HIP_TRY(d_mem.reserve(n_scans));
+  HIP_TRY(cntmat.reserve(static_cast<size_t>(words)));
+  HIP_TRY(d_res.reserve(2 * n_scans + 1));
+  if (passes > 1) HIP_TRY(tmp.reserve(c->n));
+  HIP_TRY(hipMemcpyAsync(d_mem.p, mem.data(), n_scans * sizeof(ndt::OrderMember), hipMemcpyHostToDevice, st));
+  HIP_TRY(ndt::launch_order_batch_radix(src, d_mem.p, static_cast<int>(n_scans), max_nb, passes, db, ppb, cntmat.p, d_res.p, d_res.p + n_scans,
+                                        tmp.p, c->sorted.p, w_one, st));
+  std::vector<unsigned> res(2 * n_scans + 1);
+  HIP_TRY(hipMemcpyAsync(res.data(), d_res.p, res.size() * sizeof(unsigned), hipMemcpyDeviceToHost, st));
+  HIP_TRY(hipStreamSynchronize(st));
+  for (size_t k = 0; k < n_scans; k++) {
+    c->scan_counts[k] = res[k];
+    c->scan_starts[k] = res[n_scans + k];
+  }
+  c->scan_starts[n_scans] = res[2 * n_scans];
+  c->n_sorted = res[2 * n_scans];
+  return NDT_OK;
+}
+
+ndt_status order_batch(ndt_context* h, DeviceCloud* c, const float4* src, const size_t* offsets, size_t n_scans, float resolution, bool w_one) {
   hipStream_t st = h->stream;
   c->scan_counts.assign(n_scans, 0);
   c->scan_starts.assign(n_scans + 1, 0);
@@ -298,7 +358,7 @@
     for (int j = 0; j < 6; j++) box[6 * k + j] = j < 3 ? std::numeric_limits<int>::max() : std::numeric_limits<int>::min();
   HIP_TRY(hipMemcpyAsync(d_off.p, off.data(), (n_scans + 1) * sizeof(int), hipMemcpyHostToDevice, st));
   HIP_TRY(hipMemcpyAsync(d_box.p, box.data(), box.size() * sizeof(int), hipMemcpyHostToDevice, st));
-  HIP_TRY(ndt::launch_scan_bboxes(c->pts.p, d_off.p, static_cast<int>(n_scans), static_cast<int>(max_scan), d_box.p, st));
+  HIP_TRY(ndt::launch_scan_bboxes(src, d_off.p, static_cast<int>(n_scans), static_cast<int>(max_scan), d_box.p, st));
   HIP_TRY(hipMemcpyAsync(box.data(), d_box.p, box.size() * sizeof(int), hipMemcpyDeviceToHost, st));
   HIP_TRY(hipStreamSynchronize(st));
   std::vector<ndt::ScanLattice> lat(n_scans);
@@ -308,7 +368,7 @@
     if (box[6 * k] > box[6 * k + 3]) continue;
     float mn[3], mx[3];
     for (int j = 0; j < 3; j++) { mn[j] = ndt::scan_bbox_decode(box[6 * k + j]); mx[j] = ndt::scan_bbox_decode(box[6 * k + 3 + j]); }
-    for (float pitch = h->resolution;; pitch *= 2.0f) {
+    for (float pitch = resolution;; pitch *= 2.0f) {
       const float inv = 1.0f / pitch;
       double cells = 1;
       int div[3];
@@ -326,8 +386,15 @@
       }
     }
   }
+  if (order_radix_on()) return order_batch_radix(h, c, src, offsets, n_scans, lat, max_scan, w_one);
+  return order_batch_chain(h, c, src, offsets, n_scans, lat, kMaxCounters);
+}
+
+static ndt_status order_batch_chain(ndt_context* h, DeviceCloud* c, const float4* src, const size_t* offsets, size_t n_scans,
+                                    std::vector<ndt::ScanLattice>& lat, double kMaxCounters) {
+  hipStream_t st = h->stream;
   DevBuf<unsigned> cell_count, totals, rank, d_starts;
-  DevBuf<int> key;
+  DevBuf<int> key, d_off;
   ChainBufs lv;
   DevBuf<ndt::ScanLattice> d_lat;
   DevBuf<long long> d_bases;
@@ -347,7 +414,7 @@
       continue;
     }
     const int ni = static_cast<int>(n_pts);
-    const float4* in = c->pts.p + first_pt;
+    const float4* in = src + first_pt;
     std::vector<int> poff(ns + 1);
     std::vector<long long> bases(ns + 1);
     size_t pass_max = 0;
@@ -394,12 +461,15 @@
   return NDT_OK;
 }
 
-ndt_status order_cloud(ndt_context* h, DeviceCloud* c, const size_t* offsets, size_t n_scans) {
+static bool ordering_enabled(size_t n, bool batch) {
   static const int mode = [] { const char* v = getenv("NDT_SORT_SOURCE"); return v ? (atoi(v) != 0 ? 1 : 0) : -1; }();
   constexpr size_t kOrderFrom = 65536;
+  return mode < 0 ? (batch || n >= kOrderFrom) : mode != 0;
+}
+
+ndt_status order_cloud(ndt_context* h, DeviceCloud* c, const size_t* offsets, size_t n_scans) {
   c->n_sorted = 0;
-  const bool enabled = mode < 0 ? (offsets != nullptr || c->n >= kOrderFrom) : mode != 0;
-  if (!enabled || c->n == 0) return NDT_OK;
+  if (!ordering_enabled(c->n, offsets != nullptr) || c->n == 0) return NDT_OK;
   HIP_TRY(c->sorted.reserve(c->n));
   if (!offsets) {
     size_t got = 0;
@@ -408,10 +478,35 @@
     if (s) return s;
     c->n_sorted = got;
   } else {
-    ndt_status s = order_batch(h, c, offsets, n_scans);
+    ndt_status s = order_batch(h, c, c->pts.p, offsets, n_scans, h->resolution, false);
     if (s) return s;
   }
   return NDT_OK;
+}
+
+ndt_status batch_cloud(ndt_context* h, const void* pts, size_t n, size_t stride, bool on_device, const size_t* offsets, size_t n_scans,
+                       float resolution, std::shared_ptr<DeviceCloud>& out) {
+  const bool direct = on_device && n > 0 && n_scans > 0 && pts && stride == sizeof(float4) && (reinterpret_cast<uintptr_t>(pts) & 15) == 0 &&
+                      n <= static_cast<size_t>(std::numeric_limits<int>::max()) && order_radix_on() && ordering_enabled(n, true);
+  if (direct) {
+    ndt_status s = ensure_device(h);
+    if (s) return s;
+    auto c = std::make_shared<DeviceCloud>();
+    c->n = n;
+    HIP_TRY(c->sorted.reserve(n));
+    s = order_batch(h, c.get(), static_cast<const float4*>(pts), offsets, n_scans, resolution, true);
+    if (s) return s;
+    if (c->n_sorted > 0) {
+      out = c;
+      return NDT_OK;
+    }
+  }
+  ndt_status s = upload_cloud(h, pts, n, stride, on_device, out);
+  if (s || n_scans == 0) return s;
+  out->n_sorted = 0;
+  if (!ordering_enabled(out->n, true) || out->n == 0) return NDT_OK;
+  HIP_TRY(out->sorted.reserve(out->n));
+  return order_batch(h, out.get(), out->pts.p, offsets, n_scans, resolution, false);
 }
 
 ndt_status cloud_use_on(ndt_handle h, DeviceCloud* c) {
diff --git a/toyslam_amd/csrc/ndt_grid_kernels.hip b/toyslam_amd/csrc/ndt_grid_kernels.hip
--- a/toyslam_amd/csrc/ndt_grid_kernels.hip
+++ b/toyslam_amd/csrc/ndt_grid_kernels.hip
@@ -787,10 +787,10 @@
 }
 
 constexpr int kColCols = 16, kColGroups = kK1Threads / kColCols, kColRows = 32;
-__global__ __launch_bounds__(kK1Threads) void k1_colscan(unsigned* __restrict__ cntmat, int B, int K, unsigned* __restrict__ total) {
+__device__ __forceinline__ void colscan_columns(unsigned* __restrict__ cntmat, int B, int K, unsigned* __restrict__ total, int first_col) {
   __shared__ unsigned s_part[kColGroups][kColCols + 1];
   const int c = threadIdx.x % kColCols, rg = threadIdx.x / kColCols;
-  const int col = blockIdx.x * kColCols + c;
+  const int col = first_col + c;
   const int R = (B + kColGroups - 1) / kColGroups;
   const int r0 = rg * R;
   unsigned v[kColRows];
@@ -817,6 +817,9 @@
     base += v[i];
   }
   if (rg == 0 && col < K) total[col] = all;
+}
+__global__ __launch_bounds__(kK1Threads) void k1_colscan(unsigned* __restrict__ cntmat, int B, int K, unsigned* __restrict__ total) {
+  colscan_columns(cntmat, B, K, total, blockIdx.x * kColCols);
 }
 
 __global__ __launch_bounds__(kK1Threads) void k1_scatter(const float4* __restrict__ pts, int n, int dense, GridGeom g, int map, int K,
@@ -903,6 +906,144 @@
     }
     __syncthreads();
     if (r0 == lo) mark(4);
+    if (r0 + kK1Round < hi) {
+      for (int k = threadIdx.x; k < K; k += kK1Threads) cursor[k] += tot[k];
+      for (int i = threadIdx.x; i < kK1Waves * K / 2; i += kK1Threads) reinterpret_cast<unsigned*>(tab)[i] = 0u;
+      __syncthreads();
+    }
+  }
+}
+
+__device__ __forceinline__ int scan_cell(const ScanLattice& L, const float4& p) {
+#pragma clang fp contract(off)
+  if (L.n_cells <= 0 || !finite3(p.x, p.y, p.z)) return -1;
+  const int i0 = static_cast<int>(floorf(p.x * L.inv_leaf)) - L.min_b[0];
+  const int i1 = static_cast<int>(floorf(p.y * L.inv_leaf)) - L.min_b[1];
+  const int i2 = static_cast<int>(floorf(p.z * L.inv_leaf)) - L.min_b[2];
+  const int cell = i0 + i1 * L.mul1 + i2 * L.mul2;
+  return (i0 >= 0 && i1 >= 0 && i2 >= 0 && cell >= 0 && cell < L.n_cells) ? cell : -1;
+}
+
+__global__ __launch_bounds__(kK1Threads) void kb_hist(const float4* __restrict__ src, const OrderMember* __restrict__ mem, int shift, int K,
+                                                      int ppb, unsigned* __restrict__ cntmat, unsigned* __restrict__ kept, int first) {
+  extern __shared__ unsigned k1_lds[];
+  __shared__ unsigned s_valid;
+  const OrderMember M = mem[blockIdx.y];
+  if (static_cast<int>(blockIdx.x) >= M.nb) return;
+  const int n = first ? M.n : min(M.n, static_cast<int>(kept[blockIdx.y]));
+  const float4* pts = src + M.in_off;
+  unsigned* h = k1_lds;
+  const int lo = static_cast<int>(min(static_cast<long long>(n), static_cast<long long>(blockIdx.x) * ppb));
+  const int hi = static_cast<int>(min(static_cast<long long>(n), static_cast<long long>(lo) + ppb));
+  for (int k = threadIdx.x; k < K; k += kK1Threads) h[k] = 0;
+  if (threadIdx.x == 0) s_valid = 0;
+  __syncthreads();
+  for (int base = lo + threadIdx.x; base < hi; base += 8 * kK1Threads) {
+    float4 p[8];
+#pragma unroll
+    for (int u = 0; u < 8; u++) {
+      const int i = base + u * kK1Threads;
+      p[u] = (i < hi) ? pts[i] : make_float4(NAN, NAN, NAN, 0.f);
+    }
+#pragma unroll
+    for (int u = 0; u < 8; u++) {
+      const int c = (base + u * kK1Threads < hi) ? scan_cell(M.lat, p[u]) : -1;
+      if (c >= 0) atomicAdd(&h[(c >> shift) & (K - 1)], 1u);
+    }
+  }
+  __syncthreads();
+  unsigned* row = cntmat + M.cnt_off + static_cast<size_t>(blockIdx.x) * K;
+  unsigned mine = 0;
+  for (int k = threadIdx.x; k < K; k += kK1Threads) {
+    row[k] = h[k];
+    mine += h[k];
+  }
+  if (first) {
+    if (mine) atomicAdd(&s_valid, mine);
+    __syncthreads();
+    if (threadIdx.x == 0 && s_valid) atomicAdd(&kept[blockIdx.y], s_valid);
+  }
+}
+
+__global__ __launch_bounds__(kK1Threads) void kb_colscan(const OrderMember* __restrict__ mem, int K, unsigned* __restrict__ cntmat) {
+  const OrderMember M = mem[blockIdx.y];
+  unsigned* cm = cntmat + M.cnt_off;
+  colscan_columns(cm, M.nb, K, cm + static_cast<size_t>(M.nb) * K, blockIdx.x * kColCols);
+}
+
+__global__ __launch_bounds__(kK1Threads) void kb_starts(const unsigned* __restrict__ kept, int n, unsigned* __restrict__ starts) {
+  __shared__ unsigned s_scan[kK1Waves];
+  block_scan_array(kept, starts, n, kK1Threads, s_scan, false);
+}
+
+__global__ __launch_bounds__(kK1Threads) void kb_scatter(const float4* __restrict__ src, const OrderMember* __restrict__ mem, int shift, int K,
+                                                         int ppb, const unsigned* __restrict__ cntmat, const unsigned* __restrict__ kept,
+                                                         const unsigned* __restrict__ starts, float4* __restrict__ dst, int first, int last,
+                                                         int w_one) {
+  extern __shared__ unsigned k1_lds[];
+  __shared__ unsigned s_scan[kK1Waves];
+  __shared__ unsigned long long s_mtab[kK1Waves * kMatchSlots];
+  const OrderMember M = mem[blockIdx.y];
+  if (static_cast<int>(blockIdx.x) >= M.nb) return;
+  const int n = first ? M.n : min(M.n, static_cast<int>(kept[blockIdx.y]));
+  const float4* pts = src + M.in_off;
+  float4* out = dst + (last ? static_cast<size_t>(starts[blockIdx.y]) : static_cast<size_t>(M.in_off));
+  const unsigned* cm = cntmat + M.cnt_off;
+  const unsigned* total = cm + static_cast<size_t>(M.nb) * K;
+  unsigned long long* mtab_all = s_mtab;
+  unsigned* cursor = k1_lds;
+  unsigned short* tot = reinterpret_cast<unsigned short*>(cursor + K + 2);
+  unsigned short* tab = tot + K;
+  const int lane = threadIdx.x & (kWave - 1), wave = threadIdx.x / kWave;
+  const int b = blockIdx.x;
+  const int kbits = k1_key_bits(K);
+  const int lo = static_cast<int>(min(static_cast<long long>(n), static_cast<long long>(b) * ppb));
+  const int hi = static_cast<int>(min(static_cast<long long>(n), static_cast<long long>(lo) + ppb));
+  for (int i = threadIdx.x; i < kK1Waves * kMatchSlots; i += kK1Threads) mtab_all[i] = 0ull;
+  for (int i = threadIdx.x; i < kK1Waves * K / 2; i += kK1Threads) reinterpret_cast<unsigned*>(tab)[i] = 0u;
+  block_scan_array(total, cursor, K, kK1Threads, s_scan, false);
+  __syncthreads();
+  for (int k = threadIdx.x; k < K; k += kK1Threads) cursor[k] += cm[static_cast<size_t>(b) * K + k];
+  __syncthreads();
+  unsigned short* row = tab + wave * K;
+  unsigned long long* mtab = mtab_all + wave * kMatchSlots;
+  for (int r0 = lo; r0 < hi; r0 += kK1Round) {
+    float4 p[8];
+    int key[8];
+    unsigned rk[8];
+#pragma unroll
+    for (int u = 0; u < 8; u++) {
+      const int i = r0 + wave * (8 * kWave) + u * kWave + lane;
+      p[u] = (i < hi) ? pts[i] : make_float4(NAN, NAN, NAN, 0.f);
+    }
+#pragma unroll
+    for (int u = 0; u < 8; u++) {
+      const int i = r0 + wave * (8 * kWave) + u * kWave + lane;
+      const int c = (i < hi) ? scan_cell(M.lat, p[u]) : -1;
+      key[u] = (c >= 0) ? ((c >> shift) & (K - 1)) : -1;
+      rk[u] = 0;
+      if (r0 + wave * (8 * kWave) + u * kWave < hi) rk[u] = wave_rank(key[u], key[u] >= 0, mtab, row, kbits);
+    }
+    __syncthreads();
+    for (int k = threadIdx.x; k < K; k += kK1Threads) {
+      unsigned s_ = 0;
+#pragma unroll
+      for (int w = 0; w < kK1Waves; w++) {
+        const unsigned t = tab[w * K + k];
+        tab[w * K + k] = static_cast<unsigned short>(s_);
+        s_ += t;
+      }
+      tot[k] = static_cast<unsigned short>(s_);
+    }
+    __syncthreads();
+#pragma unroll
+    for (int u = 0; u < 8; u++) {
+      if (key[u] >= 0) {
+        const unsigned pos = cursor[key[u]] + row[key[u]] + rk[u];
+        out[pos] = w_one ? make_float4(p[u].x, p[u].y, p[u].z, 1.0f) : p[u];
+      }
+    }
+    __syncthreads();
     if (r0 + kK1Round < hi) {
       for (int k = threadIdx.x; k < K; k += kK1Threads) cursor[k] += tot[k];
       for (int i = threadIdx.x; i < kK1Waves * K / 2; i += kK1Threads) reinterpret_cast<unsigned*>(tab)[i] = 0u;
@@ -2227,6 +2368,42 @@
   return hipGetLastError();
 }
 
+void order_batch_radix_plan(long long max_cells, size_t max_member_points, size_t total_points, int* passes_out, int* digit_bits_out, int* ppb_out) {
+  int bits = 4;
+  while ((1ll << bits) < max_cells) bits++;
+  const int passes = (bits + 10) / 11, db = (bits + passes - 1) / passes;
+  size_t ppb = kK1Round;
+  while (ppb < 4 * static_cast<size_t>(kK1Round) && total_points / ppb > 1024) ppb *= 2;
+  while ((max_member_points + ppb - 1) / ppb > static_cast<size_t>(kColGroups * kColRows)) ppb += kK1Round;
+  if (passes_out) *passes_out = passes;
+  if (digit_bits_out) *digit_bits_out = db;
+  if (ppb_out) *ppb_out = static_cast<int>(ppb);
+}
+hipError_t launch_order_batch_radix(const float4* src, const OrderMember* d_mem, int n_members, int max_blocks, int passes, int digit_bits,
+                                    int ppb, unsigned* cntmat, unsigned* kept, unsigned* starts, float4* tmp, float4* out, bool w_one,
+                                    hipStream_t stream) {
+  if (n_members <= 0 || max_blocks <= 0) return hipSuccess;
+  const int K = 1 << digit_bits;
+  const size_t lds_scatter = (static_cast<size_t>(K) + 2) * sizeof(unsigned) + static_cast<size_t>(K) * sizeof(unsigned short) +
+                             static_cast<size_t>(kK1Waves) * K * sizeof(unsigned short);
+  if (n_members > 65535 || digit_bits < 4 || digit_bits > 11 || max_blocks > kColGroups * kColRows || ppb % kK1Round) return hipErrorInvalidValue;
+  hipError_t e = hipMemsetAsync(kept, 0, static_cast<size_t>(n_members) * sizeof(unsigned), stream);
+  if (e != hipSuccess) return e;
+  const float4* in = src;
+  for (int p = 0; p < passes; p++) {
+    const bool last = p == passes - 1;
+    float4* dst = ((passes - p) & 1) ? out : tmp;
+    hipLaunchKernelGGL(kb_hist, dim3(max_blocks, n_members), dim3(kK1Threads), static_cast<size_t>(K) * sizeof(unsigned), stream, in, d_mem,
+                       p * digit_bits, K, ppb, cntmat, kept, p == 0 ? 1 : 0);
+    hipLaunchKernelGGL(kb_colscan, dim3((K + kColCols - 1) / kColCols, n_members), dim3(kK1Threads), 0, stream, d_mem, K, cntmat);
+    if (p == 0) hipLaunchKernelGGL(kb_starts, dim3(1), dim3(kK1Threads), 0, stream, kept, n_members, starts);
+    hipLaunchKernelGGL(kb_scatter, dim3(max_blocks, n_members), dim3(kK1Threads), lds_scatter, stream, in, d_mem, p * digit_bits, K, ppb, cntmat,
+                       kept, starts, dst, p == 0 ? 1 : 0, last ? 1 : 0, (w_one && p == 0) ? 1 : 0);
+    in = dst;
+  }
+  return hipGetLastError();
+}
+
 constexpr int kRcPrefixTiles = 2048;
 static int rc_items(long long lut_cells) {
   int items = 1;
diff --git a/toyslam_amd/csrc/ndt_handle.hip b/toyslam_amd/csrc/ndt_handle.hip
--- a/toyslam_amd/csrc/ndt_handle.hip
+++ b/toyslam_amd/csrc/ndt_handle.hip
@@ -385,16 +385,20 @@
   }
   h->profiling = on == 1;
   h->profile_server = on == 2;
+  h->profile_prepare = on == 3;
   return NDT_OK;
 }
 
 ndt_status ndt_profile_read(ndt_handle h, int kind, long long* n_launches, double* total_ms, int reset) {
-  if (!h || kind < 0 || kind >= ndt_context::kProfSlots) return fail(NDT_ERR_INVALID, "bad arguments");
-  if (n_launches) *n_launches = h->prof_n[kind];
-  if (total_ms) *total_ms = h->prof_ms[kind];
+  if (!h || kind < 0 || kind >= ndt_context::kProfSlots + 2) return fail(NDT_ERR_INVALID, "bad arguments");
+  const bool prep = kind >= ndt_context::kProfSlots;
+  long long& n = prep ? h->prep_n[kind - ndt_context::kProfSlots] : h->prof_n[kind];
+  double& ms = prep ? h->prep_ms[kind - ndt_context::kProfSlots] : h->prof_ms[kind];
+  if (n_launches) *n_launches = n;
+  if (total_ms) *total_ms = ms;
   if (reset) {
-    h->prof_n[kind] = 0;
-    h->prof_ms[kind] = 0;
+    n = 0;
+    ms = 0;
   }
   return NDT_OK;
 }
diff --git a/toyslam_amd/csrc/ndt_internal.hpp b/toyslam_amd/csrc/ndt_internal.hpp
--- a/toyslam_amd/csrc/ndt_internal.hpp
+++ b/toyslam_amd/csrc/ndt_internal.hpp
@@ -399,6 +399,10 @@
   size_t exp_voxels = 0, exp_points = 0, exp_launches = 0;
   size_t cf_launches = 0, cf_passes = 0, cf_max_blocks = 0;
   float cf_excursion = 0.f;
+  bool profile_prepare = false;
+  hipEvent_t ev_p0 = nullptr, ev_p1 = nullptr;
+  long long prep_n[2] = {0, 0};
+  double prep_ms[2] = {0, 0};
 
   ~ndt_context() {
     for (ndt_context* w : batch_workers) delete w;
@@ -449,6 +453,8 @@
     if (ev_b) (void)hipEventDestroy(ev_b);
     if (ev_c) (void)hipEventDestroy(ev_c);
     if (ev_d) (void)hipEventDestroy(ev_d);
+    if (ev_p0) (void)hipEventDestroy(ev_p0);
+    if (ev_p1) (void)hipEventDestroy(ev_p1);
     for (hipStream_t& ps : partition_stream) {
       if (ps && ps != stream) {
         DevPool::instance().forget_stream(ps);
@@ -486,7 +492,9 @@
 ndt_status bbox_compute(ndt_context* h, const float4* d_pts, int n, int dense, BBox& out);
 ndt_status order_range(ndt_context* h, const float4* d_pts, size_t n, float pitch, float4* d_out, size_t* n_out,
                        const BBox* known_bbox = nullptr);
-ndt_status order_batch(ndt_context* h, DeviceCloud* c, const size_t* offsets, size_t n_scans);
+ndt_status order_batch(ndt_context* h, DeviceCloud* c, const float4* src, const size_t* offsets, size_t n_scans, float resolution, bool w_one);
+ndt_status batch_cloud(ndt_context* h, const void* pts, size_t n, size_t stride, bool on_device, const size_t* offsets, size_t n_scans,
+                       float resolution, std::shared_ptr<DeviceCloud>& out);
 ndt_status order_cloud(ndt_context* h, DeviceCloud* c, const size_t* offsets, size_t n_scans);
 ndt_status download_records(ndt_context* h, const float4* d_src, size_t n, void* out, size_t out_stride);
 ndt_status out_block_at_least(ndt_context* h, size_t bytes);
diff --git a/toyslam_amd/csrc/ndt_kernels.hpp b/toyslam_amd/csrc/ndt_kernels.hpp
--- a/toyslam_amd/csrc/ndt_kernels.hpp
+++ b/toyslam_amd/csrc/ndt_kernels.hpp
@@ -209,6 +209,15 @@
 float scan_bbox_decode(int v);
 hipError_t launch_count_batch(const float4* pts, const int* d_scan_off, int n_scans, int max_scan_points, const ScanLattice* d_lat,
                               int* d_key, unsigned* d_rank, unsigned* d_cell_count, hipStream_t stream);
+struct OrderMember {
+  ScanLattice lat;
+  int in_off, n, nb;
+  unsigned long long cnt_off;
+};
+void order_batch_radix_plan(long long max_cells, size_t max_member_points, size_t total_points, int* passes, int* digit_bits, int* ppb);
+hipError_t launch_order_batch_radix(const float4* src, const OrderMember* d_mem, int n_members, int max_blocks, int passes, int digit_bits,
+                                    int ppb, unsigned* cntmat, unsigned* kept, unsigned* starts, float4* tmp, float4* out, bool w_one,
+                                    hipStream_t stream);
 hipError_t launch_pick(const unsigned* cell_count, const long long* d_bases, unsigned* d_out, int n, hipStream_t stream);
 hipError_t launch_scan_reduce(const unsigned* d_cell_count, long long n_cells, int min_pts, unsigned* d_block_sums,
                               int n_tiles, hipStream_t stream);
diff --git a/toyslam_amd/ndt.py b/toyslam_amd/ndt.py
--- a/toyslam_amd/ndt.py
+++ b/toyslam_amd/ndt.py
@@ -511,6 +511,33 @@
                  _f(g) if g is not None else None, _f(T), _i(conv), _i(it), _d(tp)))
         return dict(T=np.stack([_from_colmajor(T[k]) for k in range(B)]), converged=conv.astype(bool),
                     iterations=it, trans_probability=tp)
+
+    def batchOrder(self, clouds=None, resolution=None, device_ptr=None, offsets=None, stride_bytes=16):
+        if clouds is not None:
+            cat = _cloud(np.concatenate(clouds, axis=0)) if clouds else np.zeros((0, 4), np.float32)
+            offsets = np.zeros(len(clouds) + 1, dtype=np.uintp)
+            offsets[1:] = np.cumsum([c.shape[0] for c in clouds])
+            ptr, stride, on_device = cat.ctypes.data, cat.shape[1] * 4, 0
+        else:
+            offsets = np.ascontiguousarray(offsets, dtype=np.uintp)
+            ptr, stride, on_device = C.c_void_p(device_ptr), stride_bytes, 1
+        B = len(offsets) - 1
+        n_pts = int(offsets[B] - offsets[0])
+        out = np.zeros((max(n_pts, 1), 4), dtype=np.float32)
+        starts = np.zeros(B + 1, dtype=np.uintp)
+        counts = np.zeros(max(B, 1), dtype=np.uintp)
+        n = C.c_size_t(0)
+        szp = C.POINTER(C.c_size_t)
+        check(self._L.ndt_diag_batch_order(self._h, ptr, offsets.ctypes.data_as(szp), B, stride, on_device,
+                                           float(self.getResolution() if resolution is None else resolution), out.ctypes.data,
+                                           starts.ctypes.data_as(szp), counts.ctypes.data_as(szp), C.byref(n)))
+        return dict(points=out[:n.value].copy(), starts=starts.astype(np.int64), counts=counts[:B].astype(np.int64))
+
+    @staticmethod
+    def orderBatchPlan(max_cells, max_member_points, total_points):
+        p, d, b = C.c_int(0), C.c_int(0), C.c_int(0)
+        _lib.lib().ndt_host_order_batch_plan(int(max_cells), int(max_member_points), int(total_points), C.byref(p), C.byref(d), C.byref(b))
+        return dict(passes=p.value, digit_bits=d.value, points_per_block=b.value)
 
     def alignPairs(self, clouds, pairs=None, guesses=None, is_dense=True):
         resident = [isinstance(c, DeviceCloud) for c in clouds]
```

Measured after the change: 2195 registrations/s. 1.2% lower.
